# jwliao1209/DiffMusic

Measured on AMD Instinct MI355X. Metric: denoising steps/sec (10 s clip, 200-step DPS), higher is better.
Workload: dtype f16; 1 GPU; MusicLDM + DPS music_inpainting, 10 s @16 kHz, 200-step schedule, batch 8 per GPU (BASELINE.json configs[1]); global_batch=8, clips_per_gpu=8, lanes=1, parallelism=clip-sharded x1 (RCCL world size 1, no per-step collective), finite=True, nan_steps=0, settle_steps=10, cached_reference_transform=True, launched_by=single process

## Files before the change

diffmusic_amd/_lib.py:

```python
import ctypes as C
import os

_HERE = os.path.dirname(os.path.abspath(__file__))
LIB_PATH = os.environ.get("DMX_LIB_PATH") or os.path.join(_HERE, "lib", "libdiffmusic_hip.so")
MAX_STAGES = 8


class HifiGanConfig(C.Structure):
    _fields_ = [("model_in_dim", C.c_int), ("upsample_initial_channel", C.c_int), ("num_upsamples", C.c_int),
                ("upsample_rates", C.c_int * MAX_STAGES), ("upsample_kernel_sizes", C.c_int * MAX_STAGES),
                ("num_kernels", C.c_int), ("resblock_kernel_sizes", C.c_int * MAX_STAGES),
                ("num_dilations", C.c_int), ("resblock_dilation_sizes", C.c_int * (MAX_STAGES * MAX_STAGES)),
                ("leaky_relu_slope", C.c_float)]


class VaeConfig(C.Structure):
    _fields_ = [("latent_channels", C.c_int), ("out_channels", C.c_int), ("num_blocks", C.c_int),
                ("block_out_channels", C.c_int * MAX_STAGES), ("layers_per_block", C.c_int),
                ("norm_num_groups", C.c_int), ("eps", C.c_float)]


class UNetConfig(C.Structure):
    _fields_ = [("in_channels", C.c_int), ("out_channels", C.c_int), ("num_blocks", C.c_int),
                ("block_out_channels", C.c_int * MAX_STAGES), ("layers_per_block", C.c_int),
                ("attention_heads", C.c_int), ("norm_num_groups", C.c_int),
                ("down_attn", C.c_int * MAX_STAGES), ("up_attn", C.c_int * MAX_STAGES),
                ("class_embed_dim", C.c_int), ("num_attn_per_layer", C.c_int), ("attn_cross_dims", C.c_int * 4)]


class HtsatConfig(C.Structure):
    _fields_ = [("spec_size", C.c_int), ("num_mel_bins", C.c_int), ("patch_size", C.c_int), ("embed_dim", C.c_int), ("window_size", C.c_int),
                ("num_stages", C.c_int), ("depths", C.c_int * 4), ("num_heads", C.c_int * 4), ("ln_eps", C.c_float), ("bn_eps", C.c_float)]


class GemmDesc(C.Structure):
    _fields_ = [("A", C.c_void_p), ("W", C.c_void_p), ("C", C.c_void_p), ("C2", C.c_void_p),
                ("bias", C.c_void_p), ("rowbias", C.c_void_p), ("R", C.c_void_p), ("X", C.c_void_p),
                ("M", C.c_int), ("N", C.c_int), ("K", C.c_int), ("ldw", C.c_int),
                ("Hi", C.c_int), ("Wi", C.c_int), ("Ci", C.c_int), ("lda", C.c_int),
                ("Hq", C.c_int), ("Wq", C.c_int), ("sy", C.c_int), ("sx", C.c_int),
                ("ntaps", C.c_int),
                ("Ho", C.c_int), ("Wo", C.c_int), ("ldc", C.c_int), ("osy", C.c_int), ("ooy", C.c_int),
                ("osx", C.c_int), ("oox", C.c_int),
                ("ldr", C.c_int), ("ldx", C.c_int), ("ldc2", C.c_int),
                ("Z", C.c_int), ("Zi", C.c_int),
                ("sAo", C.c_longlong), ("sAi", C.c_longlong), ("sWo", C.c_longlong), ("sWi", C.c_longlong),
                ("sCo", C.c_longlong), ("sCi", C.c_longlong),
                ("alpha", C.c_float), ("act_slope", C.c_float), ("mask_slope", C.c_float),
                ("flags", C.c_int),
                ("tdy", C.c_byte * 16), ("tdx", C.c_byte * 16), ("resid_inv_slope", C.c_float), ("tile_cfg", C.c_int), ("ldrb", C.c_int), ("ksplit", C.c_int),
                ("XB", C.c_void_p), ("B2", C.c_void_p), ("ldxb", C.c_int), ("ldb2", C.c_int),
                ("colsum", C.c_void_p), ("ln_eps", C.c_float), ("rowstats_in", C.c_void_p), ("rowstats_out", C.c_void_p), ("nslots", C.c_int),
                ("gn_part", C.c_void_p), ("gnb_x", C.c_void_p), ("gnb_scale", C.c_void_p), ("gnb_shift", C.c_void_p),
                ("gnb_ldx", C.c_int), ("gnb_silu", C.c_int), ("gnb_stats", C.c_void_p), ("gnb_cpg", C.c_int)]


EPI_BIAS, EPI_ROWBIAS, EPI_RESID, EPI_ACCUM, EPI_MASK, EPI_LRELU2, EPI_TANH, EPI_F32OUT, EPI_NO_C, EPI_RESID_INV, EPI_MASKBITS, EPI_BITS2, EPI_SOFTBWD = \
    1, 2, 4, 8, 16, 32, 64, 128, 256, 512, 1024, 2048, 4096
EPI_GEGLU, EPI_LNFOLD, EPI_ROWSTATS, EPI_GNSTATS, EPI_GNBWD = 8192, 16384, 32768, 65536, 131072

_SIGS = {
    "dmx_abi_version": (C.c_int, []),
    "dmx_act_dtype": (C.c_int, []),
    "dmx_last_error": (C.c_char_p, []),
    "dmx_hifigan_create": (C.c_void_p, [C.POINTER(HifiGanConfig)]),
    "dmx_vae_decoder_create": (C.c_void_p, [C.POINTER(VaeConfig)]),
    "dmx_unet_create": (C.c_void_p, [C.POINTER(UNetConfig)]),
    "dmx_model_destroy": (None, [C.c_void_p]),
    "dmx_model_num_params": (C.c_int, [C.c_void_p]),
    "dmx_model_param_name": (C.c_char_p, [C.c_void_p, C.c_int]),
    "dmx_model_param_numel": (C.c_size_t, [C.c_void_p, C.c_int]),
    "dmx_model_param_ndim": (C.c_int, [C.c_void_p, C.c_int]),
    "dmx_model_param_dim": (C.c_int, [C.c_void_p, C.c_int, C.c_int]),
    "dmx_model_load_param": (C.c_int, [C.c_void_p, C.c_char_p, C.c_void_p, C.c_size_t]),
    "dmx_model_finalize": (C.c_int, [C.c_void_p, C.c_void_p]),
    "dmx_hifigan_out_len": (C.c_int, [C.c_void_p, C.c_int]),
    "dmx_hifigan_workspace_bytes": (C.c_size_t, [C.c_void_p, C.c_int, C.c_int]),
    "dmx_hifigan_fwd": (C.c_int, [C.c_void_p, C.c_void_p, C.c_void_p, C.c_int, C.c_int, C.c_void_p, C.c_size_t, C.c_void_p]),
    "dmx_hifigan_bwd": (C.c_int, [C.c_void_p, C.c_void_p, C.c_void_p, C.c_void_p]),
    "dmx_hifigan_fwd_dead": (C.c_int, [C.c_void_p, C.c_void_p, C.c_void_p, C.c_int, C.c_int, C.c_int, C.c_int, C.c_void_p, C.c_size_t,
                                       C.c_void_p]),
    "dmx_hifigan_dead_plan": (C.c_int, [C.c_void_p, C.POINTER(C.c_int), C.POINTER(C.c_int), C.POINTER(C.c_int), C.POINTER(C.c_int), C.c_int]),
    "dmx_conv_dead_rows": (C.c_int, [C.c_int] * 9 + [C.POINTER(C.c_int), C.POINTER(C.c_int)]),
    "dmx_vae_workspace_bytes": (C.c_size_t, [C.c_void_p, C.c_int, C.c_int, C.c_int]),
    "dmx_vae_decode_fwd": (C.c_int, [C.c_void_p, C.c_void_p, C.c_float, C.c_void_p, C.c_void_p, C.c_int, C.c_int, C.c_int,
                                     C.c_int, C.c_void_p, C.c_size_t, C.c_void_p]),
    "dmx_vae_decode_bwd": (C.c_int, [C.c_void_p, C.c_void_p, C.c_float, C.c_void_p, C.c_void_p]),
    "dmx_vae_encoder_create": (C.c_void_p, [C.POINTER(VaeConfig)]),
    "dmx_vae_encoder_workspace_bytes": (C.c_size_t, [C.c_void_p, C.c_int, C.c_int, C.c_int]),
    "dmx_vae_encode_fwd": (C.c_int, [C.c_void_p, C.c_void_p, C.c_float, C.c_void_p, C.c_int, C.c_int, C.c_int, C.c_void_p, C.c_size_t,
                                     C.c_void_p]),
    "dmx_latent_init": (C.c_int, [C.c_void_p] * 6 + [C.c_int] * 3 + [C.c_float] * 3 + [C.c_void_p]),
    "dmx_conv2d_raw": (C.c_int, [C.c_void_p] * 4 + [C.c_int] * 9 + [C.c_void_p]),
    "dmx_unet_workspace_bytes": (C.c_size_t, [C.c_void_p, C.c_int, C.c_int, C.c_int]),
    "dmx_unet_fwd": (C.c_int, [C.c_void_p, C.c_void_p, C.c_void_p, C.c_void_p, C.c_void_p, C.c_int, C.c_int, C.c_int,
                               C.c_void_p, C.c_size_t, C.c_void_p]),
    "dmx_unet_fwd_ctx": (C.c_int, [C.c_void_p] * 5 + [C.c_int, C.c_void_p, C.c_int, C.c_void_p, C.c_void_p, C.c_int, C.c_int, C.c_int,
                                   C.c_void_p, C.c_size_t, C.c_void_p]),
    "dmx_unet_workspace_bytes_ctx": (C.c_size_t, [C.c_void_p, C.c_int, C.c_int, C.c_int, C.c_int, C.c_int]),
    "dmx_htsat_create": (C.c_void_p, [C.POINTER(HtsatConfig)]),
    "dmx_htsat_feature_dims": (C.c_int, [C.c_void_p, C.POINTER(C.c_int), C.POINTER(C.c_int)]),
    "dmx_htsat_workspace_bytes": (C.c_size_t, [C.c_void_p, C.c_int, C.c_int]),
    "dmx_htsat_fwd": (C.c_int, [C.c_void_p, C.c_void_p, C.c_int, C.c_int, C.c_void_p, C.c_int, C.c_void_p, C.c_size_t, C.c_void_p]),
    "dmx_htsat_bwd": (C.c_int, [C.c_void_p, C.c_void_p, C.c_void_p, C.c_void_p, C.c_void_p]),
    "dmx_htsat_tape_raw": (C.c_size_t, [C.c_void_p, C.c_int, C.c_int, C.c_int, C.c_void_p, C.c_size_t, C.c_void_p]),
    "dmx_htsat_ln_rows_fwd_raw": (C.c_int, [C.c_void_p] * 4 + [C.c_longlong] + [C.c_int] * 4 + [C.c_float, C.c_int, C.c_void_p]),
    "dmx_htsat_ln_rows_bwd_raw": (C.c_int, [C.c_void_p] * 5 + [C.c_longlong] + [C.c_int] * 4 + [C.c_float, C.c_int, C.c_void_p]),
    "dmx_htsat_gelu_fwd_raw": (C.c_int, [C.c_void_p, C.c_void_p, C.c_longlong, C.c_void_p]),
    "dmx_htsat_gelu_bwd_raw": (C.c_int, [C.c_void_p, C.c_void_p, C.c_void_p, C.c_longlong, C.c_void_p]),
    "dmx_htsat_win_attn_fwd_raw": (C.c_int, [C.c_void_p] * 3 + [C.c_int] * 6 + [C.c_void_p]),
    "dmx_htsat_win_attn_bwd_raw": (C.c_int, [C.c_void_p] * 4 + [C.c_int] * 6 + [C.c_void_p]),
    "dmx_htsat_embed_fwd_raw": (C.c_int, [C.c_void_p, C.c_void_p, C.c_int, C.c_int, C.c_void_p, C.c_void_p]),
    "dmx_htsat_embed_bwd_raw": (C.c_int, [C.c_void_p, C.c_void_p, C.c_int, C.c_int] + [C.c_void_p] * 5),
    "dmx_gram_fwd": (C.c_int, [C.c_void_p, C.c_void_p, C.c_int, C.c_int, C.c_int, C.c_void_p]),
    "dmx_gram_bwd": (C.c_int, [C.c_void_p, C.c_void_p, C.c_void_p, C.c_int, C.c_int, C.c_int, C.c_void_p]),
    "dmx_gemm_raw": (C.c_int, [C.c_void_p, C.c_size_t, C.c_void_p]),
    "dmx_gemm_slab_eligible": (C.c_int, [C.c_void_p, C.c_size_t]),
    "dmx_gemm_last_cfg_raw": (C.c_int, []),
    "dmx_prof_begin": (None, []),
    "dmx_prof_end": (C.c_int, [C.POINTER(C.c_double), C.POINTER(C.c_double)]),
    "dmx_flash_attn_raw": (C.c_int, [C.c_void_p, C.c_void_p, C.c_void_p, C.c_void_p, C.c_void_p] + [C.c_int] * 6 + [C.c_float, C.c_void_p]),
    "dmx_flash_attn_ld_raw": (C.c_int, [C.c_void_p] * 5 + [C.c_int] * 8 + [C.c_float, C.POINTER(C.c_int), C.c_void_p]),
    "dmx_softmax_raw": (C.c_int, [C.c_void_p] * 3 + [C.c_longlong, C.c_int, C.c_longlong, C.c_longlong, C.c_int, C.c_void_p]),
    "dmx_softmax_act_raw": (C.c_int, [C.c_void_p] * 3 + [C.c_longlong, C.c_int, C.c_longlong, C.c_int, C.c_void_p]),
    "dmx_transpose_raw": (C.c_int, [C.c_void_p, C.c_void_p, C.c_int, C.c_int, C.c_longlong, C.c_longlong, C.c_int, C.c_int] + [C.c_longlong] * 4
                          + [C.c_void_p]),
    "dmx_rowdot_raw": (C.c_int, [C.c_void_p] * 3 + [C.c_longlong, C.c_int, C.c_longlong, C.c_longlong, C.c_void_p]),
    "dmx_layernorm_raw": (C.c_int, [C.c_void_p] * 4 + [C.c_int, C.c_int, C.c_float, C.c_void_p]),
    "dmx_geglu_raw": (C.c_int, [C.c_void_p, C.c_void_p, C.c_longlong, C.c_int, C.c_void_p]),
    "dmx_gemm_splitk_workspace": (C.c_int, [C.c_void_p, C.c_size_t]),
    "dmx_conv_pair_raw": (C.c_int, [C.c_void_p, C.c_void_p, C.c_size_t, C.c_void_p]),
    "dmx_conv_pair_group_raw": (C.c_int, [C.c_int, C.c_void_p, C.c_void_p, C.c_size_t, C.c_void_p]),
    "dmx_conv_pair_dead_raw": (C.c_int, [C.c_void_p, C.c_void_p, C.c_size_t, C.POINTER(C.c_int), C.POINTER(C.c_int), C.POINTER(C.c_int), C.c_void_p]),
    "dmx_conv_pair_group_dead_raw": (C.c_int, [C.c_int, C.c_void_p, C.c_void_p, C.c_size_t, C.POINTER(C.c_int), C.c_void_p]),
    "dmx_groupnorm_scratch_floats": (C.c_size_t, [C.c_int, C.c_int, C.c_int]),
    "dmx_groupnorm_raw": (C.c_int, [C.c_void_p] * 8 + [C.c_int] * 4 + [C.c_float, C.c_int, C.c_void_p]),
    "dmx_groupnorm_part_floats": (C.c_size_t, [C.c_int, C.c_int, C.c_int]),
    "dmx_groupnorm_parts_raw": (C.c_int, [C.c_void_p] * 7 + [C.c_int] * 4 + [C.c_float, C.c_int, C.c_int, C.c_void_p, C.c_void_p, C.c_void_p]),
    "dmx_gemm_last_tile_rows_raw": (C.c_int, []),
    "dmx_groupnorm_bwd_raw": (C.c_int, [C.c_void_p] * 10 + [C.c_int] * 6 + [C.c_void_p, C.c_void_p, C.c_void_p]),
    "dmx_prof_dominant": (C.c_int, [C.POINTER(C.c_double)] * 3),
    "dmx_audio_create": (C.c_void_p, [C.c_int, C.c_int, C.c_int, C.c_int, C.c_void_p]),
    "dmx_audio_destroy": (None, [C.c_void_p]),
    "dmx_audio_num_frames": (C.c_int, [C.c_void_p, C.c_int]),
    "dmx_audio_num_bins": (C.c_int, [C.c_void_p]),
    "dmx_audio_state_bytes": (C.c_size_t, [C.c_void_p, C.c_int, C.c_int]),
    "dmx_audio_transform_fwd": (C.c_int, [C.c_void_p, C.c_void_p, C.c_longlong, C.c_void_p, C.c_void_p, C.c_int, C.c_int, C.c_int,
                                          C.c_int, C.c_float, C.c_float, C.c_void_p]),
    "dmx_audio_transform_bwd": (C.c_int, [C.c_void_p, C.c_void_p, C.c_void_p, C.c_longlong, C.c_void_p, C.c_int, C.c_int, C.c_int,
                                          C.c_int, C.c_float, C.c_float, C.c_int, C.c_void_p]),
    "dmx_audio_is_fused": (C.c_int, [C.c_void_p, C.c_int]),
    "dmx_audio_guidance_fwd": (C.c_int, [C.c_void_p, C.c_void_p, C.c_longlong, C.c_void_p, C.c_void_p, C.c_longlong, C.c_void_p, C.c_void_p,
                                         C.c_int, C.c_int, C.c_int, C.c_int, C.c_float, C.c_float, C.c_void_p]),
    "dmx_audio_guidance_bwd": (C.c_int, [C.c_void_p, C.c_void_p, C.c_longlong, C.c_void_p, C.c_void_p, C.c_longlong, C.c_float, C.c_void_p,
                                         C.c_void_p, C.c_longlong, C.c_int, C.c_void_p, C.c_int, C.c_int, C.c_int, C.c_int, C.c_float, C.c_float,
                                         C.c_void_p]),
    "dmx_audio_guidance_fwd_ex": (C.c_int, [C.c_void_p, C.c_void_p, C.c_longlong, C.c_void_p, C.c_void_p, C.c_longlong, C.c_void_p, C.c_void_p,
                                            C.c_int, C.c_int, C.c_int, C.c_int, C.c_float, C.c_float, C.c_void_p, C.c_longlong, C.c_void_p,
                                            C.c_float, C.c_void_p]),
    "dmx_audio_guidance_bwd_ex": (C.c_int, [C.c_void_p, C.c_void_p, C.c_longlong, C.c_void_p, C.c_void_p, C.c_longlong, C.c_float, C.c_void_p,
                                            C.c_void_p, C.c_longlong, C.c_int, C.c_void_p, C.c_int, C.c_int, C.c_int, C.c_int, C.c_float, C.c_float,
                                            C.c_void_p, C.c_longlong, C.c_void_p, C.c_float, C.c_void_p]),
    "dmx_audio_guidance_fwd_shaped": (C.c_int, [C.c_void_p, C.c_void_p, C.c_longlong, C.c_void_p, C.c_void_p, C.c_longlong, C.c_void_p, C.c_void_p,
                                                C.c_int, C.c_int, C.c_int, C.c_int, C.c_float, C.c_float, C.c_void_p, C.c_longlong, C.c_void_p,
                                                C.c_float, C.c_void_p, C.c_void_p]),
    "dmx_audio_guidance_bwd_shaped": (C.c_int, [C.c_void_p, C.c_void_p, C.c_longlong, C.c_void_p, C.c_void_p, C.c_longlong, C.c_float, C.c_void_p,
                                                C.c_void_p, C.c_longlong, C.c_int, C.c_void_p, C.c_int, C.c_int, C.c_int, C.c_int, C.c_float, C.c_float,
                                                C.c_void_p, C.c_longlong, C.c_void_p, C.c_float, C.c_void_p, C.c_void_p]),
    "dmx_clip_fwd": (C.c_int, [C.c_void_p, C.c_longlong, C.c_void_p, C.c_void_p, C.c_longlong, C.c_int, C.c_int, C.c_void_p]),
    "dmx_clip_bwd": (C.c_int, [C.c_void_p, C.c_longlong, C.c_void_p, C.c_longlong, C.c_void_p, C.c_void_p, C.c_longlong, C.c_int, C.c_int, C.c_int,
                               C.c_void_p]),
    "dmx_declip_project": (C.c_int, [C.c_void_p, C.c_longlong, C.c_void_p, C.c_longlong, C.c_void_p, C.c_void_p, C.c_longlong, C.c_int, C.c_int,
                                     C.c_void_p]),
    "dmx_drc_fwd": (C.c_int, [C.c_void_p, C.c_longlong, C.c_void_p, C.c_longlong, C.c_void_p, C.c_void_p, C.c_int, C.c_int] + [C.c_float] * 6 +
                    [C.c_void_p]),
    "dmx_drc_bwd": (C.c_int, [C.c_void_p, C.c_longlong, C.c_void_p, C.c_longlong, C.c_void_p, C.c_void_p, C.c_void_p, C.c_void_p, C.c_longlong,
                              C.c_int, C.c_int, C.c_int] + [C.c_float] * 6 + [C.c_void_p]),
    "dmx_drc_fwd_p": (C.c_int, [C.c_void_p, C.c_longlong, C.c_void_p, C.c_longlong, C.c_void_p, C.c_void_p, C.c_void_p, C.c_int, C.c_int, C.c_float,
                                C.c_void_p]),
    "dmx_drc_bwd_p": (C.c_int, [C.c_void_p, C.c_longlong, C.c_void_p, C.c_longlong] + [C.c_void_p] * 6 + [C.c_longlong, C.c_int, C.c_int, C.c_int,
                                                                                                        C.c_float, C.c_void_p]),
    "dmx_drc_pgrad": (C.c_int, [C.c_void_p] * 6 + [C.c_int, C.c_int, C.c_float, C.c_void_p]),
    "dmx_drc_update": (C.c_int, [C.c_void_p] * 5 + [C.c_int] * 3 + [C.c_void_p] + [C.c_double] * 3 + [C.c_float, C.c_void_p, C.c_void_p, C.c_void_p]),
    "dmx_warp_fwd": (C.c_int, [C.c_void_p, C.c_longlong, C.c_void_p, C.c_longlong, C.c_void_p, C.c_int, C.c_int, C.c_void_p]),
    "dmx_warp_bwd": (C.c_int, [C.c_void_p, C.c_void_p, C.c_longlong, C.c_void_p, C.c_int, C.c_int, C.c_int, C.c_void_p]),
    "dmx_warp_wgrad": (C.c_int, [C.c_void_p, C.c_void_p, C.c_longlong, C.c_void_p, C.c_longlong, C.c_void_p, C.c_int, C.c_int, C.c_void_p]),
    "dmx_warp_update": (C.c_int, [C.c_void_p] * 5 + [C.c_int] * 4 + [C.c_double] * 5 + [C.c_int, C.c_void_p]),
    "dmx_click_detect": (C.c_int, [C.c_void_p, C.c_longlong] + [C.c_void_p] * 5 + [C.c_int, C.c_int, C.c_float, C.c_float, C.c_void_p]),
    "dmx_click_mask": (C.c_int, [C.c_void_p, C.c_void_p, C.c_void_p, C.c_int, C.c_int, C.c_int, C.c_void_p]),
    "dmx_mask_rows": (C.c_int, [C.c_void_p, C.c_longlong, C.c_void_p, C.c_longlong, C.c_void_p, C.c_int, C.c_int, C.c_int, C.c_void_p]),
    "dmx_declick_blend": (C.c_int, [C.c_void_p, C.c_longlong, C.c_void_p, C.c_longlong, C.c_void_p, C.c_longlong, C.c_void_p, C.c_int, C.c_int,
                                    C.c_int, C.c_void_p]),
    "dmx_noise_add": (C.c_int, [C.c_void_p, C.c_void_p, C.c_void_p, C.c_longlong, C.c_float, C.c_void_p]),
    "dmx_audio_stft_mag": (C.c_int, [C.c_void_p, C.c_void_p, C.c_longlong, C.c_void_p, C.c_void_p, C.c_int, C.c_int, C.c_void_p]),
    "dmx_audio_stft_mag_bwd": (C.c_int, [C.c_void_p, C.c_void_p, C.c_void_p, C.c_longlong, C.c_void_p, C.c_int, C.c_int, C.c_int, C.c_void_p]),
    "dmx_audio_tf_frames": (C.c_int, [C.c_int]),
    "dmx_audio_tf_gain": (C.c_int, [C.c_void_p, C.c_void_p, C.c_longlong, C.c_void_p, C.c_longlong, C.c_void_p, C.c_longlong, C.c_int, C.c_int, C.c_int,
                                    C.c_void_p]),
    "dmx_audio_tf_curve": (C.c_int, [C.c_void_p, C.c_void_p, C.c_longlong, C.c_void_p, C.c_longlong, C.c_void_p, C.c_longlong, C.c_int, C.c_int, C.c_int,
                                     C.c_void_p]),
    "dmx_audio_tf_wgrad_segments": (C.c_int, [C.c_int]),
    "dmx_audio_tf_wgrad": (C.c_int, [C.c_void_p, C.c_void_p, C.c_longlong, C.c_void_p, C.c_longlong, C.c_void_p, C.c_int, C.c_int, C.c_void_p]),
    "dmx_audio_eq_update": (C.c_int, [C.c_void_p, C.c_int] + [C.c_void_p] * 3 + [C.c_int, C.c_int] + [C.c_double] * 4 + [C.c_int, C.c_void_p]),
    "dmx_mdct_frames": (C.c_int, [C.c_int]),
    "dmx_mdct_quant": (C.c_int, [C.c_void_p, C.c_void_p, C.c_longlong, C.c_void_p, C.c_longlong, C.c_void_p, C.c_void_p, C.c_longlong, C.c_int, C.c_int,
                                 C.c_int, C.c_int, C.c_void_p]),
    "dmx_mdct_project": (C.c_int, [C.c_void_p, C.c_void_p, C.c_longlong, C.c_void_p, C.c_longlong, C.c_void_p, C.c_void_p, C.c_longlong, C.c_int,
                                   C.c_int, C.c_int, C.c_void_p]),
    "dmx_audio_melscale": (C.c_int, [C.c_void_p, C.c_void_p, C.c_void_p, C.c_int, C.c_int, C.c_float, C.c_float, C.c_void_p]),
    "dmx_mask_apply": (C.c_int, [C.c_void_p, C.c_longlong, C.c_void_p, C.c_void_p, C.c_longlong, C.c_int, C.c_int, C.c_int, C.c_void_p]),
    "dmx_l2_loss": (C.c_int, [C.c_void_p, C.c_longlong, C.c_void_p, C.c_void_p, C.c_void_p, C.c_int, C.c_longlong, C.c_float, C.c_void_p]),
    "dmx_track_stitch_fwd": (C.c_int, [C.c_void_p, C.c_longlong, C.c_void_p, C.POINTER(C.c_int)] + [C.c_int] * 4 + [C.c_void_p]),
    "dmx_track_stitch_bwd": (C.c_int, [C.c_void_p, C.c_void_p, C.c_longlong, C.POINTER(C.c_int)] + [C.c_int] * 5 + [C.c_void_p]),
    "dmx_stem_mix_fwd": (C.c_int, [C.c_void_p, C.c_longlong, C.c_void_p, C.POINTER(C.c_float)] + [C.c_int] * 3 + [C.c_void_p]),
    "dmx_stem_mix_bwd": (C.c_int, [C.c_void_p, C.c_void_p, C.c_longlong, C.POINTER(C.c_float)] + [C.c_int] * 4 + [C.c_void_p]),
    "dmx_stem_project": (C.c_int, [C.c_void_p, C.c_longlong, C.c_void_p, C.c_void_p, C.POINTER(C.c_float), C.c_int, C.c_int, C.c_void_p]),
    "dmx_grad_normalize": (C.c_int, [C.c_void_p, C.c_void_p, C.c_int, C.c_longlong, C.c_float, C.c_void_p]),
    "dmx_fir_fwd": (C.c_int, [C.c_void_p, C.c_longlong, C.c_void_p, C.c_void_p, C.c_longlong] + [C.c_int] * 7 + [C.c_void_p]),
    "dmx_fir_bwd": (C.c_int, [C.c_void_p, C.c_longlong, C.c_void_p, C.c_void_p, C.c_void_p, C.c_longlong] + [C.c_int] * 7 + [C.c_void_p]),
    "dmx_fir_clip_fwd": (C.c_int, [C.c_void_p, C.c_longlong, C.c_void_p, C.c_void_p, C.c_longlong] + [C.c_int] * 4 + [C.c_void_p]),
    "dmx_fir_clip_bwd": (C.c_int, [C.c_void_p, C.c_longlong, C.c_void_p, C.c_void_p, C.c_void_p, C.c_longlong] + [C.c_int] * 4 + [C.c_void_p]),
    "dmx_fir_wgrad_workspace_floats": (C.c_size_t, [C.c_int, C.c_int, C.c_int]),
    "dmx_fir_wgrad": (C.c_int, [C.c_void_p, C.c_longlong, C.c_void_p, C.c_longlong, C.c_void_p, C.c_size_t] + [C.c_int] * 4 + [C.c_void_p]),
    "dmx_ir_update": (C.c_int, [C.c_void_p, C.c_int] + [C.c_void_p] * 4 + [C.c_int, C.c_int] + [C.c_double] * 4 + [C.c_int, C.c_void_p]),
    "dmx_sched_pred_x0": (C.c_int, [C.c_void_p, C.c_void_p, C.c_void_p, C.c_longlong, C.c_float, C.c_void_p]),
    "dmx_sched_pred_x0_ex": (C.c_int, [C.c_void_p, C.c_void_p, C.c_void_p, C.c_longlong, C.c_float, C.c_int, C.c_float, C.c_void_p]),
    "dmx_sched_step_ex": (C.c_int, [C.c_int] + [C.c_void_p] * 9 + [C.c_int, C.c_int] + [C.c_float] * 5 + [C.c_int, C.c_int, C.c_float, C.c_void_p]),
    "dmx_sched_cfg_combine": (C.c_int, [C.c_void_p, C.c_void_p, C.c_longlong, C.c_float, C.c_void_p]),
    "dmx_randn_philox": (C.c_int, [C.c_void_p, C.c_int, C.c_longlong, C.POINTER(C.c_ulonglong), C.c_ulonglong, C.c_void_p]),
    "dmx_sched_step": (C.c_int, [C.c_int] + [C.c_void_p] * 9 + [C.c_int, C.c_int] + [C.c_float] * 5 + [C.c_int, C.c_void_p]),
}

ADDED_IN_V4 = ("dmx_vae_encoder_create", "dmx_vae_encoder_workspace_bytes", "dmx_vae_encode_fwd", "dmx_latent_init",
               "dmx_track_stitch_fwd", "dmx_track_stitch_bwd", "dmx_audio_guidance_fwd_shaped", "dmx_audio_guidance_bwd_shaped",
               "dmx_clip_fwd", "dmx_clip_bwd", "dmx_declip_project", "dmx_hifigan_fwd_dead", "dmx_hifigan_dead_plan", "dmx_conv_dead_rows",
               "dmx_fir_clip_fwd", "dmx_fir_clip_bwd", "dmx_fir_wgrad", "dmx_fir_wgrad_workspace_floats", "dmx_ir_update",
               "dmx_stem_mix_fwd", "dmx_stem_mix_bwd", "dmx_stem_project", "dmx_audio_tf_gain", "dmx_audio_tf_frames",
               "dmx_audio_tf_curve", "dmx_audio_tf_wgrad_segments", "dmx_audio_tf_wgrad", "dmx_audio_eq_update", "dmx_drc_fwd", "dmx_drc_bwd",
               "dmx_warp_fwd", "dmx_warp_bwd", "dmx_warp_wgrad", "dmx_warp_update", "dmx_drc_fwd_p", "dmx_drc_bwd_p", "dmx_drc_pgrad",
               "dmx_drc_update", "dmx_click_detect", "dmx_click_mask", "dmx_mask_rows", "dmx_declick_blend", "dmx_mdct_frames",
               "dmx_mdct_quant", "dmx_mdct_project")

_lib = None


def check_symbols(h, path=LIB_PATH):
    for name in ADDED_IN_V4:
        if not hasattr(h, name):
            raise RuntimeError(f"{path} reports ABI version {ABI_VERSION} but does not export `{name}` (a build from before the VAE "
                               "encoder / track-mode / declipping / blind-dereverberation / source-separation / time-frequency-masking / blind-equalisation / de-compression / wow-and-flutter / blind-wow-and-flutter / blind-de-compression / declicking / codec-restoration entry points): rebuild it (python -m diffmusic_amd.build --force)")


def lib():
    global _lib
    if _lib is None:
        if not os.path.exists(LIB_PATH):
            raise RuntimeError(f"{LIB_PATH} is missing: build it with `python -m diffmusic_amd.build` "
                               "(the diffmusic_amd hot path has no CPU fallback)")
        h = C.CDLL(LIB_PATH)
        for name, (res, args) in _SIGS.items():
            if not hasattr(h, name):
                continue
            fn = getattr(h, name)
            fn.restype, fn.argtypes = res, args
        if h.dmx_abi_version() != ABI_VERSION:
            raise RuntimeError(f"libdiffmusic_hip.so ABI version {h.dmx_abi_version()} != {ABI_VERSION} expected by this package: rebuild it "
                               "(python -m diffmusic_amd.build --force)")
        check_symbols(h)
        _lib = h
    return _lib


ABI_VERSION = 4


def act_dtype():
    import torch
    return torch.float16 if lib().dmx_act_dtype() == 1 else torch.bfloat16


class DmxError(RuntimeError):
    pass


def check(rc, what=""):
    if rc != 0:
        msg = lib().dmx_last_error()
        raise DmxError(f"{what} failed with code {rc}: {msg.decode() if msg else ''}")
```

diffmusic_amd/csrc/blocks.h:

```cpp
#pragma once
#include <cstdlib>
#include "models.h"

struct Ctx {
  Arena* arena;
  hipStream_t st;
  bool dry;
  float* gn_partial;
  bool gn_parts = true;
};
#define CRUN(expr) do { if (!cx.dry) { int rc_ = (expr); if (rc_ != DMX_OK) return rc_; } } while (0)
#define CTRY(expr) do { int rc__ = (expr); if (rc__ != DMX_OK) return rc__; } while (0)

struct GnTape { float* stats = nullptr; float* scale = nullptr; float* shift = nullptr; };

inline bool gn_parts_wanted(const Ctx& cx, size_t P) {
  const bool on = cx.gn_parts && getenv("DMX_NO_GN_PARTS") == nullptr;
  return on && P > 512;
}
inline float* gn_part_alloc(Ctx& cx, int B, size_t P, int Np) { return cx.arena->f32(dmx_gn_part_floats(B, (int)P, Np)); }
inline void gn_parts_push(Ctx& cx, GnParts* gp, float* buf, int tm, int P, int Np, int Creal, int qoff = 0) {
  if (!gp || gp->n < 0) return;
  if (cx.dry) tm = 32;
  if (tm > 0 && gp->n < 8) gp->r[gp->n++] = GnRegion{buf, tm, P, Np / 4, qoff, Creal / 4};
  else gp->n = -1;
}
inline GnParts gn_parts_concat(const GnParts& a, const GnParts& b, int Ca) {
  GnParts o;
  if (a.n <= 0 || b.n <= 0 || a.n + b.n > 8) { o.n = -1; return o; }
  for (int i = 0; i < a.n; ++i) o.r[o.n++] = a.r[i];
  for (int i = 0; i < b.n; ++i) { o.r[o.n] = b.r[i]; o.r[o.n++].qoff += Ca / 4; }
  return o;
}
inline const GnParts* gn_parts_valid(const GnParts* p) { return p && p->n > 0 ? p : nullptr; }
inline GnParts gn_parts_new(Ctx& cx, int B, size_t P, int Np) {
  GnParts g;
  if (gn_parts_wanted(cx, P)) g.r[0].part = gn_part_alloc(cx, B, P, Np); else g.n = -1;
  return g;
}
inline float* gn_parts_buf(const GnParts& g) { return g.n == 0 ? g.r[0].part : nullptr; }

inline int conv_fwd_2d_gn(Ctx& cx, const ConvLayer& L, const act_t* in, void* out, int B, int H, int W, Epi e, GnParts* out_parts, int Creal) {
  float* buf = out_parts ? gn_parts_buf(*out_parts) : nullptr;
  e.gn_part = buf;
  int rows = 0;
  CRUN(conv_fwd_2d(L, in, out, B, H, W, e, cx.st, &rows));
  const int Ho = (H + L.pad_h + L.pad_h_hi - L.kh) / L.stride + 1, Wo = (W + L.pad_w + L.pad_w_hi - L.kw) / L.stride + 1;
  if (buf) gn_parts_push(cx, out_parts, buf, rows, Ho * Wo, L.Cop, Creal);
  return DMX_OK;
}

inline int upsample_conv_fwd_gn(Ctx& cx, const ConvLayer& L, const act_t* x, act_t* y, int B, int H, int W, int H2, int W2, int C, bool fold,
                                GnParts* out_parts) {
  Arena& A = *cx.arena;
  const size_t P = (size_t)H * W, P2 = (size_t)H2 * W2;
  GnParts up;
  float* ubuf[4] = {nullptr, nullptr, nullptr, nullptr};
  if (gn_parts_wanted(cx, P2)) for (int q = 0; q < (fold ? 4 : 1); ++q) ubuf[q] = gn_part_alloc(cx, B, fold ? P : P2, L.Cop);
  else up.n = -1;
  const size_t mk = A.mark();
  Epi e;
  if (fold) {
    int rows[4] = {0, 0, 0, 0};
    CRUN(conv_up2x_fwd(L, x, y, B, H, W, e, cx.st, ubuf[0] ? ubuf : nullptr, rows));
    if (ubuf[0]) for (int q = 0; q < 4; ++q) gn_parts_push(cx, &up, ubuf[q], rows[q], (int)P, L.Cop, C);
  } else {
    act_t* u = A.bf(B * P2 * C);
    CRUN(dmx_upsample_nearest(x, u, B, H, W, H2, W2, C, cx.st));
    up.r[0].part = ubuf[0];
    CTRY(conv_fwd_2d_gn(cx, L, u, y, B, H2, W2, e, &up, C));
  }
  A.release(mk);
  *out_parts = up;
  return DMX_OK;
}

struct GnLayer {
  GroupNormLayer g;
  const float* gamma = nullptr;
  const float* beta = nullptr;
  void build(ParamStore& ps, const std::string& pre, int C, int G, float eps) { g = make_gn(ps, pre, C, G, eps); }
  void bind(ParamStore& ps) { gamma = ps.dev(g.g_id); beta = ps.dev(g.b_id); }
  GnTape alloc(Ctx& cx, int B) const {
    GnTape t;
    t.stats = cx.arena->f32((size_t)B * g.G * 2);
    t.scale = cx.arena->f32((size_t)B * g.C);
    t.shift = cx.arena->f32((size_t)B * g.C);
    return t;
  }
  int fwd(Ctx& cx, const act_t* x, act_t* y, int B, int P, int silu, const GnTape& t, const GnParts* parts = nullptr) const {
    CRUN(dmx_groupnorm_fwd(x, y, gamma, beta, t.stats, t.scale, t.shift, cx.gn_partial, B, P, g.C, g.G, g.eps, silu, cx.st,
                           gn_parts_valid(parts)));
    return DMX_OK;
  }
  int conv_bwd_2d_gn(Ctx& cx, const ConvLayer& L, const act_t* dout, act_t* dy, int B, int H, int W, const act_t* x, int silu, const GnTape& t,
                     GnParts* bparts) const {
    const size_t P = (size_t)H * W;
    GnParts gp;
    Epi e;
    int rows = 0;
    if (!gn_parts_wanted(cx, P) || ((g.C / g.G) & 3) || (g.C & 7) || getenv("DMX_NO_GN_BWD_PARTS")) {
      gp.n = -1;
    } else {
      e.gn_part = gn_part_alloc(cx, B, P, g.C);
      e.gnb_x = x; e.gnb_scale = t.scale; e.gnb_shift = t.shift; e.gnb_silu = silu; e.gnb_stats = t.stats; e.gnb_cpg = g.C / g.G;
    }
    CRUN(conv_bwd_2d(L, dout, dy, B, H, W, e, cx.st, &rows));
    if (e.gn_part) gn_parts_push(cx, &gp, e.gn_part, rows, (int)P, g.C, g.C);
    *bparts = gp;
    return DMX_OK;
  }
  int bwd(Ctx& cx, const act_t* x, const act_t* dy, const act_t* add, act_t* dx, int B, int P, int silu, const GnTape& t,
          const GnParts* bparts = nullptr) const {
    const size_t mk = cx.arena->mark();
    float* k0 = cx.arena->f32((size_t)B * g.C);
    float* k1 = cx.arena->f32((size_t)B * g.C);
    CRUN(dmx_groupnorm_bwd(x, dy, add, dx, t.stats, t.scale, t.shift, k0, k1, cx.gn_partial, B, P, g.C, g.G, silu, cx.st,
                           gn_parts_valid(bparts)));
    cx.arena->release(mk);
    return DMX_OK;
  }
};

struct ResnetTape { const act_t* x = nullptr; act_t* h1 = nullptr; GnTape g1, g2; };

struct Resnet2D {
  int Cin = 0, Cout = 0;
  GnLayer norm1, norm2;
  ConvLayer conv1, conv2, shortcut, temb;
  bool has_shortcut = false, has_temb = false;

  void build(ParamStore& ps, const std::string& pre, int cin, int cout, int temb_ch, int groups, float eps, bool need_bwd) {
    Cin = cin; Cout = cout;
    norm1.build(ps, pre + ".norm1", cin, groups, eps);
    conv1 = make_conv2d(ps, pre + ".conv1", cin, cout, 3, 1, 1, need_bwd);
    if (temb_ch > 0) { temb = make_linear(ps, pre + ".time_emb_proj", temb_ch, cout, true, false); has_temb = true; }
    norm2.build(ps, pre + ".norm2", cout, groups, eps);
    conv2 = make_conv2d(ps, pre + ".conv2", cout, cout, 3, 1, 1, need_bwd);
    if (cin != cout) { shortcut = make_conv2d(ps, pre + ".conv_shortcut", cin, cout, 1, 1, 0, need_bwd); has_shortcut = true; }
  }
  int pack(ParamStore& ps, hipStream_t st) {
    norm1.bind(ps); norm2.bind(ps);
    CTRY(pack_layer(ps, conv1, st));
    CTRY(pack_layer(ps, conv2, st));
    if (has_shortcut) CTRY(pack_layer(ps, shortcut, st));
    if (has_temb) CTRY(pack_layer(ps, temb, st));
    return DMX_OK;
  }
  int fwd(Ctx& cx, const act_t* x, act_t* out, int B, int H, int W, const act_t* silu_emb, ResnetTape* tape,
          const float* rb_pre = nullptr, int ldrb = 0, const GnParts* x_parts = nullptr, GnParts* out_parts = nullptr) const {
    Arena& A = *cx.arena;
    const size_t P = (size_t)H * W;
    ResnetTape t;
    t.x = x;
    if (tape) { t.h1 = A.bf(B * P * Cout); t.g1 = norm1.alloc(cx, B); t.g2 = norm2.alloc(cx, B); }
    const size_t mk = A.mark();
    if (!tape) { t.h1 = A.bf(B * P * Cout); t.g1 = norm1.alloc(cx, B); t.g2 = norm2.alloc(cx, B); }
    act_t* n = A.bf(B * P * (Cin > Cout ? Cin : Cout));
    CTRY(norm1.fwd(cx, x, n, B, (int)P, 1, t.g1, x_parts));
    Epi e1;
    GnParts h1p = gn_parts_new(cx, B, P, conv1.Cop);
    if (has_temb && rb_pre) {
      e1.flags = EPI_ROWBIAS; e1.rowbias = rb_pre; e1.ldrb = ldrb;
    } else if (has_temb) {
      float* rb = A.f32((size_t)B * Cout);
      Epi et; et.flags = EPI_F32OUT;
      CRUN(linear_fwd(temb, silu_emb, temb.Cip, rb, Cout, B, et, cx.st));
      e1.flags = EPI_ROWBIAS; e1.rowbias = rb;
    }
    CTRY(conv_fwd_2d_gn(cx, conv1, n, t.h1, B, H, W, e1, &h1p, Cout));
    CTRY(norm2.fwd(cx, t.h1, n, B, (int)P, 1, t.g2, &h1p));
    Epi e2; e2.flags = EPI_RESID; e2.R = x;
    if (has_shortcut) {
      act_t* sc = A.bf(B * P * Cout);
      Epi es;
      CRUN(conv_fwd_2d(shortcut, x, sc, B, H, W, es, cx.st));
      e2.R = sc;
    }
    CTRY(conv_fwd_2d_gn(cx, conv2, n, out, B, H, W, e2, out_parts, Cout));
    A.release(mk);
    if (tape) *tape = t;
    return DMX_OK;
  }
  int bwd(Ctx& cx, const act_t* dout, act_t* dx, int B, int H, int W, const ResnetTape& t) const {
    Arena& A = *cx.arena;
    const size_t P = (size_t)H * W;
    const size_t mk = A.mark();
    act_t* a = A.bf(B * P * Cout);
    act_t* b = A.bf(B * P * (Cin > Cout ? Cin : Cout));
    Epi e;
    GnParts bp2, bp1;
    CTRY(norm2.conv_bwd_2d_gn(cx, conv2, dout, a, B, H, W, t.h1, 1, t.g2, &bp2));
    CTRY(norm2.bwd(cx, t.h1, a, nullptr, b, B, (int)P, 1, t.g2, &bp2));
    act_t* c = A.bf(B * P * Cin);
    CTRY(norm1.conv_bwd_2d_gn(cx, conv1, b, c, B, H, W, t.x, 1, t.g1, &bp1));
    const act_t* add = dout;
    if (has_shortcut) {
      CRUN(conv_bwd_2d(shortcut, dout, b, B, H, W, e, cx.st));
      add = b;
    }
    CTRY(norm1.bwd(cx, t.x, c, add, dx, B, (int)P, 1, t.g1, &bp1));
    A.release(mk);
    return DMX_OK;
  }
};

inline int attention_core(Ctx& cx, const act_t* q, const act_t* k, const act_t* v, act_t* o, int B, int Nq, int Nk, int C,
                          int heads, act_t* P_keep, const float* colbias, int ldq = 0, int ldk = 0, int ldv = 0) {
  if (ldq <= 0) ldq = C;
  if (ldk <= 0) ldk = C;
  if (ldv <= 0) ldv = C;
  Arena& A = *cx.arena;
  const int dh = C / heads, Z = B * heads;
  const int Nkp = pad8(Nk);
  if (dh & 7) { dmx_set_error("attention needs head_dim %% 8 == 0 (dh=%d)", dh); return DMX_ERR_SHAPE; }
  const float scale = 1.0f / sqrtf((float)dh);
  const size_t mk = A.mark();
  static const bool fused_ok = getenv("DMX_NO_FLASH") == nullptr;
  const bool flash = !P_keep && fused_ok && dmx_flash_attn_ok(dh, C);
  if (!flash && (Nk & 3)) { dmx_set_error("attention through materialised scores needs Nk %% 4 == 0 (Nk=%d)", Nk); return DMX_ERR_SHAPE; }
  if (flash) {
    CRUN(dmx_flash_attn_fwd(q, k, v, o, colbias, B, Nq, Nk, C, heads, scale, cx.st, ldq, ldk, ldv));
    A.release(mk);
    return DMX_OK;
  }
  act_t* Pm = P_keep ? P_keep : A.bf((size_t)Z * Nq * Nkp);
  act_t* vT = A.bf((size_t)Z * dh * Nkp);
  GemmBatch gb;
  gb.Z = Z; gb.Zi = heads;
  gb.sAo = (long long)Nq * ldq; gb.sAi = dh;
  gb.sBo = (long long)Nk * ldk; gb.sBi = dh;
  gb.sCo = (long long)heads * Nq * Nkp; gb.sCi = (long long)Nq * Nkp;
  Epi e; e.alpha = scale;
  CRUN(gemm_nt(q, ldq, k, ldk, Pm, Nkp, Nq, Nk, dh, e, gb, cx.st));
  CRUN(dmx_softmax_act(Pm, Pm, colbias, (long long)Z * Nq, Nk, Nkp, heads * Nq, cx.st));
  if (Nkp != Nk && !cx.dry) (void)hipMemsetAsync(vT, 0, (size_t)Z * dh * Nkp * sizeof(act_t), cx.st);
  CRUN(dmx_transpose(v, vT, Nk, dh, ldv, Nkp, Z, heads, (long long)Nk * ldv, dh, (long long)heads * dh * Nkp, (long long)dh * Nkp, cx.st));
  GemmBatch g2;
  g2.Z = Z; g2.Zi = heads;
  g2.sAo = (long long)heads * Nq * Nkp; g2.sAi = (long long)Nq * Nkp;
  g2.sBo = (long long)heads * dh * Nkp; g2.sBi = (long long)dh * Nkp;
  g2.sCo = (long long)Nq * C; g2.sCi = dh;
  Epi e2;
  CRUN(gemm_nt(Pm, Nkp, vT, Nkp, o, C, Nq, dh, Nkp, e2, g2, cx.st));
  A.release(mk);
  return DMX_OK;
}

struct VaeMidAttention {
  int C = 0;
  bool need_bwd = false;
  GnLayer norm;
  ConvLayer to_q, to_k, to_v, to_out;
  GnTape t_norm;
  const act_t* x_in = nullptr;
  act_t *q = nullptr, *k = nullptr, *v = nullptr, *Pm = nullptr, *O = nullptr;

  void build(ParamStore& ps, const std::string& pre, int C_, int G, float eps, bool need_bwd_) {
    C = C_; need_bwd = need_bwd_;
    norm.build(ps, pre + ".group_norm", C, G, eps);
    to_q = make_linear(ps, pre + ".to_q", C, C, true, need_bwd);
    to_k = make_linear(ps, pre + ".to_k", C, C, true, need_bwd);
    to_v = make_linear(ps, pre + ".to_v", C, C, true, need_bwd);
    to_out = make_linear(ps, pre + ".to_out.0", C, C, true, need_bwd);
  }
  int pack(ParamStore& ps, hipStream_t st) {
    norm.bind(ps);
    CTRY(pack_layer(ps, to_q, st));
    CTRY(pack_layer(ps, to_k, st));
    CTRY(pack_layer(ps, to_v, st));
    CTRY(pack_layer(ps, to_out, st));
    return DMX_OK;
  }
  int fwd(Ctx& cx, const act_t* x, act_t** out, int B, int H, int W, bool keep, const GnParts* x_parts, GnParts* out_parts) {
    Arena& A = *cx.arena;
    const int N = H * W;
    const size_t n = (size_t)B * N * C;
    x_in = x;
    t_norm = norm.alloc(cx, B);
    if (need_bwd) { q = A.bf(n); k = A.bf(n); v = A.bf(n); }
    Pm = keep ? A.bf((size_t)B * N * pad8(N)) : nullptr;
    O = keep ? A.bf(n) : nullptr;
    act_t* y = A.bf(n);
    GnParts op = gn_parts_new(cx, B, (size_t)N, pad8(C));
    const size_t mk = A.mark();
    act_t* xn = A.bf(n);
    if (!need_bwd) { q = A.bf(n); k = A.bf(n); v = A.bf(n); }
    act_t* o = keep ? O : A.bf(n);
    CTRY(norm.fwd(cx, x, xn, B, N, 0, t_norm, x_parts));
    Epi e;
    CRUN(linear_fwd(to_q, xn, C, q, C, (long long)B * N, e, cx.st));
    CRUN(linear_fwd(to_k, xn, C, k, C, (long long)B * N, e, cx.st));
    CRUN(linear_fwd(to_v, xn, C, v, C, (long long)B * N, e, cx.st));
    CTRY(attention_core(cx, q, k, v, o, B, N, N, C, 1, Pm, nullptr));
    Epi er; er.flags = EPI_RESID; er.R = x;
    if (gn_parts_buf(op)) CTRY(conv_fwd_2d_gn(cx, to_out, o, y, B, H, W, er, &op, C));
    else CRUN(linear_fwd(to_out, o, C, y, C, (long long)B * N, er, cx.st));
    A.release(mk);
    *out = y; *out_parts = op;
    return DMX_OK;
  }
  int bwd(Ctx& cx, const act_t* g, act_t* gx, int B, int H, int W) const {
    Arena& A = *cx.arena;
    const int N = H * W;
    hipStream_t st = cx.st;
    if (N & 7) { dmx_set_error("vae attention backward needs h*w %% 8 == 0"); return DMX_ERR_SHAPE; }
    if ((long long)B * N * C >= (1ll << 29)) { dmx_set_error("vae attention backward: B*h*w*C >= 2^29 elements unsupported"); return DMX_ERR_SHAPE; }
    const float scale = 1.0f / sqrtf((float)C);
    const size_t mk = A.mark();
    act_t* go = A.bf((size_t)B * N * C);
    act_t* goT = A.bf((size_t)B * N * C);
    act_t* PT = A.bf((size_t)B * N * N);
    float* delta = A.f32((size_t)B * N);
    act_t* dS = A.bf((size_t)B * N * N);
    act_t* T1 = A.bf((size_t)B * N * C);
    act_t* gq = A.bf((size_t)B * N * C);
    act_t* gk = A.bf((size_t)B * N * C);
    act_t* gv = A.bf((size_t)B * N * C);
    act_t* gxn = A.bf((size_t)B * N * C);
    Epi e;
    CRUN(linear_bwd(to_out, g, C, go, C, (long long)B * N, e, st));
    GemmBatch gb; gb.Z = B; gb.Zi = 1;
    CRUN(dmx_rowdot(go, O, delta, (long long)B * N, C, C, C, st));
    gb.sAo = (long long)N * C; gb.sBo = (long long)N * C; gb.sCo = (long long)N * N;
    {
      Epi es; es.flags = EPI_SOFTBWD; es.X = Pm; es.rowbias = delta; es.alpha = scale;
      CRUN(gemm_nt(go, C, v, C, dS, N, N, N, C, es, gb, st));
    }
    CRUN(dmx_transpose(Pm, PT, N, N, N, N, B, 1, (long long)N * N, 0, (long long)N * N, 0, st));
    CRUN(dmx_transpose(go, goT, N, C, C, N, B, 1, (long long)N * C, 0, (long long)N * C, 0, st));
    gb.sAo = (long long)N * N; gb.sBo = (long long)N * C; gb.sCo = (long long)N * C;
    CRUN(gemm_nt(PT, N, goT, N, gv, C, N, C, N, e, gb, st));
    CRUN(dmx_transpose(k, T1, N, C, C, N, B, 1, (long long)N * C, 0, (long long)N * C, 0, st));
    CRUN(gemm_nt(dS, N, T1, N, gq, C, N, C, N, e, gb, st));
    CRUN(dmx_transpose(dS, PT, N, N, N, N, B, 1, (long long)N * N, 0, (long long)N * N, 0, st));
    CRUN(dmx_transpose(q, T1, N, C, C, N, B, 1, (long long)N * C, 0, (long long)N * C, 0, st));
    CRUN(gemm_nt(PT, N, T1, N, gk, C, N, C, N, e, gb, st));
    Epi ea; ea.flags = EPI_ACCUM;
    CRUN(linear_bwd(to_q, gq, C, gxn, C, (long long)B * N, e, st));
    CRUN(linear_bwd(to_k, gk, C, gxn, C, (long long)B * N, ea, st));
    CRUN(linear_bwd(to_v, gv, C, gxn, C, (long long)B * N, ea, st));
    CTRY(norm.bwd(cx, x_in, gxn, g, gx, B, N, 0, t_norm));
    A.release(mk);
    return DMX_OK;
  }
};
```

diffmusic_amd/csrc/dmx_common.h:

```cpp
#pragma once
#include <hip/hip_runtime.h>
#include <stdint.h>
#include <stddef.h>

typedef uint16_t act_t;

#define DMX_OK 0
#define DMX_ERR_SHAPE (-1)
#define DMX_ERR_WORKSPACE (-2)
#define DMX_ERR_PARAM (-3)
#define DMX_ERR_STATE (-4)
#define DMX_ERR_LAUNCH (-5)

typedef __attribute__((ext_vector_type(4))) float f32x4;
#ifdef DMX_BF16
typedef __bf16 native16_t;
typedef __attribute__((ext_vector_type(8))) __bf16 frag8_t;
#define DMX_MFMA16(a, b, c) __builtin_amdgcn_mfma_f32_16x16x32_bf16(a, b, c, 0, 0, 0)
#define DMX_ACT_DTYPE 0
#else
typedef _Float16 native16_t;
typedef __attribute__((ext_vector_type(8))) _Float16 frag8_t;
#define DMX_MFMA16(a, b, c) __builtin_amdgcn_mfma_f32_16x16x32_f16(a, b, c, 0, 0, 0)
#define DMX_ACT_DTYPE 1
#endif

__device__ __forceinline__ float a2f(act_t v) { return (float)__builtin_bit_cast(native16_t, v); }
__device__ __forceinline__ act_t f2a(float f) { return __builtin_bit_cast(act_t, (native16_t)f); }
#ifdef DMX_BF16
__device__ __forceinline__ uint32_t pack2a(float lo, float hi) { return (uint32_t)f2a(lo) | ((uint32_t)f2a(hi) << 16); }
#else
__device__ __forceinline__ uint32_t pack2a(float lo, float hi) {
  typedef float dmx_f32x2 __attribute__((ext_vector_type(2)));
  typedef _Float16 dmx_f16x2 __attribute__((ext_vector_type(2)));
  const dmx_f32x2 v = {lo, hi};
  return __builtin_bit_cast(uint32_t, __builtin_convertvector(v, dmx_f16x2));
}
#endif
__device__ __forceinline__ float alo(uint32_t u) { return a2f((act_t)(u & 0xffffu)); }
__device__ __forceinline__ float ahi(uint32_t u) { return a2f((act_t)(u >> 16)); }

__device__ __forceinline__ float wave_sum(float v) {
#pragma unroll
  for (int o = 32; o > 0; o >>= 1) v += __shfl_xor(v, o, 64);
  return v;
}
__device__ __forceinline__ float wave_max(float v) {
#pragma unroll
  for (int o = 32; o > 0; o >>= 1) v = fmaxf(v, __shfl_xor(v, o, 64));
  return v;
}
__device__ __forceinline__ float block_sum(float v, float* sh) {
  v = wave_sum(v);
  const int w = threadIdx.x >> 6, nw = blockDim.x >> 6;
  __syncthreads();
  if ((threadIdx.x & 63) == 0) sh[w] = v;
  __syncthreads();
  float r = 0.f;
  for (int i = 0; i < nw; ++i) r += sh[i];
  return r;
}
__device__ __forceinline__ float block_max(float v, float* sh) {
  v = wave_max(v);
  const int w = threadIdx.x >> 6, nw = blockDim.x >> 6;
  __syncthreads();
  if ((threadIdx.x & 63) == 0) sh[w] = v;
  __syncthreads();
  float r = -3.0e38f;
  for (int i = 0; i < nw; ++i) r = fmaxf(r, sh[i]);
  return r;
}

static inline int cdiv(int a, int b) { return (a + b - 1) / b; }
static inline size_t align_up(size_t v, size_t a) { return (v + a - 1) / a * a; }

#define DMX_MAX_TAPS 16
enum {
  EPI_BIAS = 1,
  EPI_ROWBIAS = 2,
  EPI_RESID = 4,
  EPI_ACCUM = 8,
  EPI_MASK = 16,
  EPI_LRELU2 = 32,
  EPI_TANH = 64,
  EPI_F32OUT = 128,
  EPI_NO_C = 256,
  EPI_RESID_INV = 512,
  EPI_MASKBITS = 1024,
  EPI_BITS2 = 2048,
  EPI_GEGLU = 8192,
  EPI_LNFOLD = 16384,
  EPI_ROWSTATS = 32768,
  EPI_GNSTATS = 65536,
  EPI_GNBWD = 131072,
  EPI_BIASINIT = 262144,
  EPI_SOFTBWD = 4096
};

struct GemmDesc {
  const act_t* A;
  const act_t* W;
  void* C;
  act_t* C2;
  const float* bias;
  const float* rowbias;
  const act_t* R;
  const act_t* X;
  int M, N, K;
  int ldw;
  int Hi, Wi, Ci, lda;
  int Hq, Wq, sy, sx;
  int ntaps;
  int Ho, Wo, ldc, osy, ooy, osx, oox;
  int ldr, ldx, ldc2;
  int Z, Zi;
  long long sAo, sAi, sWo, sWi, sCo, sCi;
  float alpha, act_slope, mask_slope;
  int flags;
  signed char tdy[DMX_MAX_TAPS], tdx[DMX_MAX_TAPS];
  float resid_inv_slope;
  int tile_cfg;
  int ldrb;
  int ksplit;
  const unsigned char* XB;
  unsigned char* B2;
  int ldxb, ldb2;
  const float* colsum;
  float ln_eps;
  const float* rowstats_in;
  float* rowstats_out;
  int nslots;
  float* gn_part;
  const act_t* gnb_x;
  const float* gnb_scale;
  const float* gnb_shift;
  int gnb_ldx, gnb_silu;
  const float* gnb_stats;
  int gnb_cpg;
};

int dmx_gemm_launch(const GemmDesc& d, hipStream_t stream, int* gn_rows = nullptr);
void dmx_gemm_set_splitk_workspace(float* ws, size_t bytes);
void dmx_gemm_release_splitk_workspace(const float* ws);
int dmx_gemm_launch_ln(int cfg, const GemmDesc& d, hipStream_t stream);
int dmx_gemm_launch_rowstats(int cfg, const GemmDesc& d, hipStream_t stream);
int dmx_gemm_launch_gnstats(int cfg, const GemmDesc& d, hipStream_t stream, int* gn_rows);
bool dmx_prof_is_active();
bool dmx_gemm_slab_ok(const GemmDesc& d);
int dmx_gemm_last_cfg();
```

diffmusic_amd/csrc/gemm_conv.hip:

```cpp
#include "gemm_tile.h"

namespace {
template <int BM, int BN, int WM, int WN, int NSTAGE>
int launch_glds(const GemmDesc& d, hipStream_t stream) {
  if (d.flags & EPI_SOFTBWD) {
    if constexpr (BM == 256 && BN == 256) return launch_glds_t<BM, BN, WM, WN, NSTAGE, 2>(d, stream);
    else return DMX_ERR_SHAPE;
  }
  if (d.flags & EPI_GEGLU) return launch_glds_t<BM, BN, WM, WN, NSTAGE, 3>(d, stream);
  return (d.flags & (EPI_MASKBITS | EPI_BITS2)) ? launch_glds_t<BM, BN, WM, WN, NSTAGE, 1>(d, stream)
                                                : launch_glds_t<BM, BN, WM, WN, NSTAGE, 0>(d, stream);
}

template <int S>
int launch_slab(const GemmDesc& d, hipStream_t stream) {
  return (d.flags & (EPI_MASKBITS | EPI_BITS2)) ? launch_glds_t<320, 256, 2, 4, 2, 1, false, S>(d, stream)
                                                : launch_glds_t<320, 256, 2, 4, 2, 0, false, S>(d, stream);
}

template <int BM, int BN, int WM, int WN>
int launch_cfg(const GemmDesc& d, hipStream_t stream) {
  if (d.flags & EPI_SOFTBWD) return DMX_ERR_SHAPE;
  if (d.flags & EPI_GEGLU) {
    if constexpr ((BN / WN) % 32 == 0) return launch_cfg_t<BM, BN, WM, WN, 3>(d, stream);
    else return DMX_ERR_SHAPE;
  }
  return (d.flags & (EPI_MASKBITS | EPI_BITS2)) ? launch_cfg_t<BM, BN, WM, WN, 1>(d, stream) : launch_cfg_t<BM, BN, WM, WN, 0>(d, stream);
}

}

#include <vector>
#include <cstdio>
#include <cstdlib>
#include <cmath>
namespace {
struct ProfRec { hipEvent_t a, b; double flops, bytes; int M, N, K, Z, taps, flags, cfg; };
int g_last_cfg = 0;
bool g_prof = false;
std::vector<ProfRec> g_prof_recs;
struct TileEntry { int M, N, K, Z, cfg; };
static const TileEntry g_tile_table[] = {
#include "tile_table.inc"
    {0, 0, 0, 0, 0}};

bool glds_ok(const GemmDesc& d) {
  const long long imgs = d.Hq * d.Wq > 0 ? (d.M + (long long)d.Hq * d.Wq - 1) / ((long long)d.Hq * d.Wq) : 1;
  const long long in_elems = (d.Hi > 1 || d.ntaps > 1 ? imgs * d.Hi * d.Wi : (long long)d.M) * d.lda;
  static const bool strided_ok = getenv("DMX_NO_GLDS_STRIDED") == nullptr;
  return in_elems < (1ll << 29) && (long long)d.M * d.lda < (1ll << 29) && ((long long)d.N + 512) * d.ldw < (1ll << 29) &&
         (d.sy == 1 || strided_ok);
}
}

bool dmx_gemm_slab_ok(const GemmDesc& d) {
  if (d.Hi != 1 || d.Hq != 1 || d.sx != 1 || d.ntaps < 2 || d.ntaps > DMX_MAX_TAPS || (d.Ci & 63) || d.Ci <= 0 || d.N <= 0 || (d.N & 255)) return false;
  if (d.Wq <= 0 || d.M % d.Wq != 0 || d.ksplit > 1) return false;
  int lo = 127, hi = -128;
  for (int t = 0; t < d.ntaps; ++t) {
    if (d.tdy[t] != 0) return false;
    lo = d.tdx[t] < lo ? d.tdx[t] : lo;
    hi = d.tdx[t] > hi ? d.tdx[t] : hi;
  }
  if (hi - lo > SLAB_HALO) return false;
  if (d.flags & (EPI_F32OUT | EPI_SOFTBWD | EPI_GEGLU | EPI_LNFOLD | EPI_ROWSTATS | EPI_GNSTATS | EPI_GNBWD)) return false;
  if ((d.ldc | d.ldr | d.ldx | d.ldc2) & 7) return false;
  return glds_ok(d);
}
int dmx_gemm_last_cfg() { return g_last_cfg; }

namespace {
inline int slab_cfg(int ntaps) { return ntaps >= 6 ? 21 : (ntaps >= 3 ? 20 : 22); }
int slab_adopt(const GemmDesc& d) {
  static const bool no_slab = getenv("DMX_NO_SLAB") != nullptr;
  if (no_slab || !(d.N == 256 || d.N == 512) || !(d.ntaps == 3 || d.ntaps == 7 || d.ntaps == 11) || d.Z != 1 || !dmx_gemm_slab_ok(d)) return 7;
  const long long flat = (long long)cdiv(d.M, 320) * (d.N / 256), per_image = (long long)(d.M / d.Wq) * cdiv(d.Wq, 320) * (d.N / 256);
  return (per_image + 255) / 256 <= (flat + 255) / 256 ? slab_cfg(d.ntaps) : 7;
}

int launch_by_cfg(int cfg, const GemmDesc& d, hipStream_t stream, int* gn_rows = nullptr) {
  g_last_cfg = cfg;
  if (cfg >= 20 && cfg <= 22) {
    const int S = cfg == 20 ? 2 : (cfg == 21 ? 1 : 3);
    if (!dmx_gemm_slab_ok(d) || d.ntaps * S < 6) return DMX_ERR_SHAPE;
    return S == 2 ? launch_slab<2>(d, stream) : (S == 1 ? launch_slab<1>(d, stream) : launch_slab<3>(d, stream));
  }
  if (d.flags & EPI_LNFOLD) return dmx_gemm_launch_ln(cfg, d, stream);
  if (d.flags & EPI_ROWSTATS) return dmx_gemm_launch_rowstats(cfg, d, stream);
  if (d.flags & (EPI_GNSTATS | EPI_GNBWD)) return dmx_gemm_launch_gnstats(cfg, d, stream, gn_rows);
  switch (cfg) {
    case 1: return launch_glds<256, 256, 2, 4, 2>(d, stream);
    case 2: return launch_glds<256, 128, 4, 2, 3>(d, stream);
    case 7: return launch_glds<320, 256, 2, 4, 2>(d, stream);
    case 8: return launch_glds<192, 256, 2, 4, 2>(d, stream);
    case 9: return launch_glds<320, 128, 4, 2, 2>(d, stream);
    case 10: return launch_glds<192, 128, 4, 2, 3>(d, stream);
    case 11: return launch_glds<128, 128, 2, 2, 2>(d, stream);
    case 12: return launch_glds<64, 64, 2, 2, 4>(d, stream);
    case 13: return launch_glds<128, 64, 2, 2, 3>(d, stream);
    case 14: return launch_glds<64, 128, 2, 2, 3>(d, stream);
    case 15: return launch_glds<64, 64, 2, 2, 8>(d, stream);
    case 16: return launch_glds<64, 128, 2, 2, 6>(d, stream);
    case 17: return launch_glds<128, 64, 2, 2, 6>(d, stream);
    case 18: return launch_glds<128, 128, 2, 2, 4>(d, stream);
    case 19: return launch_glds<512, 128, 4, 2, 2>(d, stream);
    case 3: return launch_cfg<128, 128, 2, 2>(d, stream);
    case 4: return launch_cfg<128, 64, 2, 2>(d, stream);
    case 5: return launch_cfg<128, 32, 4, 1>(d, stream);
    default: return launch_cfg<64, 64, 2, 2>(d, stream);
  }
}
int launch_dispatch(const GemmDesc& d, hipStream_t stream, int* gn_rows) {
  const bool gl = glds_ok(d);
  if (d.flags & EPI_SOFTBWD) return gl ? launch_by_cfg(1, d, stream, gn_rows) : DMX_ERR_SHAPE;
  if (d.tile_cfg >= 1 && d.tile_cfg <= 22 && ((d.tile_cfg > 2 && d.tile_cfg < 7) || gl)) return launch_by_cfg(d.tile_cfg, d, stream, gn_rows);
  {
    static int ovN[8], ovC[8], nov = -1;
    if (nov < 0) {
      nov = 0;
      if (const char* e = getenv("DMX_CFG_OVERRIDE")) {
        while (*e && nov < 8) {
          int n = 0, c = 0;
          if (sscanf(e, "%d:%d", &n, &c) == 2) { ovN[nov] = n; ovC[nov] = c; ++nov; }
          while (*e && *e != ',') ++e;
          if (*e == ',') ++e;
        }
      }
    }
    if (gl && d.M >= 40000)
      for (int i = 0; i < nov; ++i) if (ovN[i] == d.N) return launch_by_cfg(ovC[i], d, stream, gn_rows);
  }
  for (const TileEntry* e = g_tile_table; e->cfg; ++e)
    if (e->M == d.M && e->N == d.N && e->K == d.K && e->Z == d.Z) {
      int c = e->cfg % 100;
      if (c == 7) c = slab_adopt(d);
      if ((c > 2 && c < 7) || gl) return launch_by_cfg(c, d, stream, gn_rows);
    }
  if (gl && d.M >= 2048 && d.N % 128 == 0) {
    auto cost = [&](int bm, int bn, int slots, double eff) {
      const double blocks = (double)cdiv(d.M, bm) * cdiv(d.N, bn) * d.Z;
      const double rounds = ceil(blocks / slots);
      return rounds * (bm / 128.0) * (bn / 128.0) * (slots / 256.0) / eff;
    };
    struct Cand { int cfg, bm, bn, slots; double eff; };
    static const Cand cands[] = {{1, 256, 256, 256, 0.95}, {7, 320, 256, 256, 0.93}, {8, 192, 256, 256, 0.88},
                                 {2, 256, 128, 256, 0.70}, {9, 320, 128, 256, 0.70}, {10, 192, 128, 256, 0.66},
                                 {19, 512, 128, 256, 0.75},
                                 {3, 128, 128, 512, 0.66}};
    int best = 0;
    double bc = 1e30;
    for (const Cand& c : cands) {
      if (c.bn == 256 && d.N % 256) continue;
      const double v = cost(c.bm, c.bn, c.slots, c.eff);
      if (v < bc) { bc = v; best = c.cfg; }
    }
    if (best == 7) best = slab_adopt(d);
    if (best && best != 3) return launch_by_cfg(best, d, stream, gn_rows);
  }
  if (d.N > 32 && (long long)cdiv(d.M, 128) * cdiv(d.N, 128) * d.Z < 200) {
    if (gl && d.K >= 512 && d.Z == 1) return launch_by_cfg(d.N % 128 == 0 && d.M >= 4000 ? 14 : 12, d, stream, gn_rows);
    return launch_by_cfg(6, d, stream, gn_rows);
  }
  if (d.N > 64) return launch_by_cfg(3, d, stream, gn_rows);
  if (d.N > 32) return launch_by_cfg(4, d, stream, gn_rows);
  return launch_by_cfg(5, d, stream, gn_rows);
}
}

bool dmx_prof_is_active() { return g_prof; }

extern "C" void dmx_prof_begin(void) {
  for (auto& r : g_prof_recs) { (void)hipEventDestroy(r.a); (void)hipEventDestroy(r.b); }
  g_prof_recs.clear();
  g_prof = true;
}
static double g_dma_ms = 0.0, g_dma_fl = 0.0, g_dma_by = 0.0;
static int g_dma_n = 0;
#ifdef DMX_GEMM_STAMPS
extern "C" int dmx_gemm_stamps_read(unsigned long long* host) {
  return hipMemcpyFromSymbol(host, HIP_SYMBOL(g_gemm_stamps), sizeof(unsigned long long) * 8192 * 6) == hipSuccess ? 0 : -1;
}
#endif

extern "C" int dmx_prof_dominant(double* ms, double* flops, double* bytes) {
  if (ms) *ms = g_dma_ms;
  if (flops) *flops = g_dma_fl;
  if (bytes) *bytes = g_dma_by;
  return g_dma_n;
}
extern "C" int dmx_prof_end(double* total_ms, double* total_flops) {
  g_prof = false;
  g_dma_ms = g_dma_fl = g_dma_by = 0.0; g_dma_n = 0;
  (void)hipDeviceSynchronize();
  double ms = 0.0, fl = 0.0;
  FILE* csv = getenv("DMX_PROF_CSV") ? fopen(getenv("DMX_PROF_CSV"), "w") : nullptr;
  if (csv) fprintf(csv, "M,N,K,Z,taps,flags,cfg,ms,tflops\n");
  for (auto& r : g_prof_recs) {
    float t = 0.f;
    if (hipEventElapsedTime(&t, r.a, r.b) == hipSuccess) ms += t;
    if (csv) fprintf(csv, "%d,%d,%d,%d,%d,%d,%d,%.4f,%.1f\n", r.M, r.N, r.K, r.Z, r.taps, r.flags, r.cfg, t, t > 0 ? r.flops / t / 1e9 : 0.0);
    const bool dma = r.cfg == 1 || r.cfg == 2 || (r.cfg >= 7 && r.cfg <= 10) || (r.cfg >= 19 && r.cfg <= 22);
    if (dma) { g_dma_ms += t; g_dma_fl += r.flops; g_dma_by += r.bytes; ++g_dma_n; }
    fl += r.flops;
    (void)hipEventDestroy(r.a); (void)hipEventDestroy(r.b);
  }
  if (csv) fclose(csv);
  const int n = (int)g_prof_recs.size();
  g_prof_recs.clear();
  if (total_ms) *total_ms = ms;
  if (total_flops) *total_flops = fl;
  return n;
}

namespace {
float* g_splitk_ws = nullptr;
size_t g_splitk_bytes = 0;

__global__ void splitk_epilogue_kernel(const GemmDesc p, const float* __restrict__ ws, int ksplit) {
  const long long q = (long long)blockIdx.x * blockDim.x + threadIdx.x;
  const int nq = p.N >> 2;
  if (q >= (long long)p.M * nq) return;
  const int m = (int)(q / nq), n = (int)(q - (long long)m * nq) * 4;
  const long long mn = (long long)p.M * p.N;
  float4 v = *reinterpret_cast<const float4*>(ws + (long long)m * p.N + n);
  for (int s = 1; s < ksplit; ++s) {
    const float4 w = *reinterpret_cast<const float4*>(ws + s * mn + (long long)m * p.N + n);
    v.x += w.x; v.y += w.y; v.z += w.z; v.w += w.w;
  }
  float a[4] = {v.x, v.y, v.z, v.w};
  const int flags = p.flags;
  const long long row = m;
  if (flags & EPI_MASK) {
    const uint2 xr = *reinterpret_cast<const uint2*>(p.X + row * p.ldx + n);
    const float x[4] = {alo(xr.x), ahi(xr.x), alo(xr.y), ahi(xr.y)};
#pragma unroll
    for (int e = 0; e < 4; ++e) a[e] *= x[e] > 0.f ? 1.f : p.mask_slope;
  }
  if (flags & EPI_BIAS) {
    const float4 bb = *reinterpret_cast<const float4*>(p.bias + n);
    a[0] += bb.x; a[1] += bb.y; a[2] += bb.z; a[3] += bb.w;
  }
  if (flags & EPI_ROWBIAS) {
    const float4 bb = *reinterpret_cast<const float4*>(p.rowbias + (long long)(m / (p.Hq * p.Wq)) * (p.ldrb ? p.ldrb : p.N) + n);
    a[0] += bb.x; a[1] += bb.y; a[2] += bb.z; a[3] += bb.w;
  }
  if (flags & EPI_RESID) {
    const uint2 rr = *reinterpret_cast<const uint2*>(p.R + row * p.ldr + n);
    const float is = (flags & EPI_RESID_INV) ? p.resid_inv_slope : 1.f;
    const float x[4] = {alo(rr.x), ahi(rr.x), alo(rr.y), ahi(rr.y)};
#pragma unroll
    for (int e = 0; e < 4; ++e) a[e] += fminf(x[e], x[e] * is);
  }
#pragma unroll
  for (int e = 0; e < 4; ++e) a[e] *= p.alpha;
  if (!(flags & EPI_NO_C))
    *reinterpret_cast<uint2*>(reinterpret_cast<act_t*>(p.C) + row * p.ldc + n) = make_uint2(pack2a(a[0], a[1]), pack2a(a[2], a[3]));
  if (flags & EPI_LRELU2) {
    const float sl = p.act_slope;
    *reinterpret_cast<uint2*>(p.C2 + row * p.ldc2 + n) =
        make_uint2(pack2a(fmaxf(a[0], a[0] * sl), fmaxf(a[1], a[1] * sl)), pack2a(fmaxf(a[2], a[2] * sl), fmaxf(a[3], a[3] * sl)));
  }
}

int splitk_plan(const GemmDesc& d, int* tile) {
  static const bool off = getenv("DMX_NO_SPLITK") != nullptr;
  if (off || !g_splitk_ws || d.Z != 1 || !glds_ok(d)) return 1;
  if (d.flags & (EPI_ACCUM | EPI_F32OUT | EPI_TANH | EPI_MASKBITS | EPI_BITS2 | EPI_SOFTBWD | EPI_GEGLU | EPI_LNFOLD | EPI_ROWSTATS)) return 1;
  if (!(d.osy == 1 && d.osx == 1 && d.ooy == 0 && d.oox == 0 && d.Ho == d.Hq && d.Wo == d.Wq)) return 1;
  if ((d.N & 7) || (d.ldc & 3)) return 1;
  const int nk = (d.K + BK - 1) / BK;
  auto fits = [&](int ks) { return ks >= 2 && ks <= nk && (size_t)ks * d.M * d.N * sizeof(float) <= g_splitk_bytes; };
  auto dma_tile = [](int t) { return t == 1 || t == 2 || (t >= 7 && t <= 19); };
  if (d.tile_cfg >= 100) { *tile = d.tile_cfg % 100; return fits(d.tile_cfg / 100) && dma_tile(*tile) ? d.tile_cfg / 100 : 1; }
  if (d.tile_cfg) return 1;
  for (const TileEntry* e = g_tile_table; e->cfg; ++e)
    if (e->M == d.M && e->N == d.N && e->K == d.K && e->Z == d.Z) {
      if (e->cfg < 100) return 1;
      *tile = e->cfg % 100;
      return fits(e->cfg / 100) && dma_tile(*tile) ? e->cfg / 100 : 1;
    }
  if (d.M > 8192) return 1;
  const long long tiles = (long long)cdiv(d.M, 64) * cdiv(d.N, 64);
  if (nk < 24 || tiles >= 256) return 1;
  int ks = (int)(1024 / tiles);
  if (ks > nk / 8) ks = nk / 8;
  if (ks > 8) ks = 8;
  while (ks > 1 && !fits(ks)) --ks;
  *tile = d.N % 128 == 0 && d.M >= 4096 ? 14 : 12;
  return ks < 2 ? 1 : ks;
}

int launch_splitk(const GemmDesc& d, int ks, int tile, hipStream_t stream) {
  GemmDesc g = d;
  g.ksplit = ks;
  g.flags = EPI_F32OUT;
  g.C = g_splitk_ws; g.C2 = nullptr; g.ldc = d.N; g.alpha = 1.f;
  g.bias = nullptr; g.rowbias = nullptr; g.R = nullptr; g.X = nullptr;
  g.Ho = d.Hq; g.Wo = d.Wq;
  g.tile_cfg = 0;
  int rc = launch_by_cfg(tile, g, stream);
  if (rc != DMX_OK) return rc;
  const long long nthr = (long long)d.M * (d.N >> 2);
  hipLaunchKernelGGL(splitk_epilogue_kernel, dim3((unsigned)((nthr + 255) / 256)), dim3(256), 0, stream, d, g_splitk_ws, ks);
  g_last_cfg = 100 * ks + tile;
  return hipGetLastError() == hipSuccess ? DMX_OK : DMX_ERR_LAUNCH;
}
}

void dmx_gemm_set_splitk_workspace(float* ws, size_t bytes) { g_splitk_ws = ws; g_splitk_bytes = bytes; }
void dmx_gemm_release_splitk_workspace(const float* ws) { if (g_splitk_ws == ws) { g_splitk_ws = nullptr; g_splitk_bytes = 0; } }

int dmx_prof_open(hipStream_t st) {
  if (!g_prof) return -1;
  ProfRec r;
  memset(&r, 0, sizeof(r));
  (void)hipEventCreate(&r.a); (void)hipEventCreate(&r.b);
  (void)hipEventRecord(r.a, st);
  g_prof_recs.push_back(r);
  return (int)g_prof_recs.size() - 1;
}
void dmx_prof_close(int rec, hipStream_t st, double flops, double bytes, int M, int N, int K, int taps, int flags, int cfg) {
  if (rec < 0 || rec >= (int)g_prof_recs.size()) return;
  ProfRec& r = g_prof_recs[rec];
  (void)hipEventRecord(r.b, st);
  r.flops = flops; r.bytes = bytes; r.M = M; r.N = N; r.K = K; r.Z = 1; r.taps = taps; r.flags = flags; r.cfg = cfg;
}

int dmx_gemm_launch(const GemmDesc& d, hipStream_t stream, int* gn_rows) {
  if (gn_rows) *gn_rows = 0;
  if (d.M <= 0 || d.N <= 0 || d.K <= 0) return DMX_ERR_SHAPE;
  if ((d.Ci & 7) || (d.N & 3) || (d.K & 7) || (d.lda & 7) || (d.ldw & 7) || (d.ldc & 3)) return DMX_ERR_SHAPE;
  if (d.ntaps < 1 || d.ntaps > DMX_MAX_TAPS || d.K != d.ntaps * d.Ci) return DMX_ERR_SHAPE;
  if (d.Z < 1 || d.Zi < 1) return DMX_ERR_SHAPE;
  if ((d.flags & EPI_LRELU2) && !(d.act_slope >= 0.f && d.act_slope <= 1.f)) return DMX_ERR_SHAPE;
  if ((d.flags & EPI_RESID_INV) && !(d.resid_inv_slope >= 1.f)) return DMX_ERR_SHAPE;
  if (d.flags & EPI_SOFTBWD) {
    if ((d.flags & ~(EPI_SOFTBWD)) || ((d.N | d.ldc | d.ldx) & 7) || !d.X || !d.rowbias || d.Zi != 1 || d.ntaps != 1) return DMX_ERR_SHAPE;
    if (!(d.osy == 1 && d.osx == 1 && d.ooy == 0 && d.oox == 0 && d.Ho == d.Hq && d.Wo == d.Wq)) return DMX_ERR_SHAPE;
  }
  if (d.flags & EPI_GEGLU) {
    if ((d.flags & ~(EPI_GEGLU | EPI_BIAS | EPI_LNFOLD)) || (d.N & 31) || (d.ldc & 7) || d.ldc < d.N / 2 || d.alpha != 1.f) return DMX_ERR_SHAPE;
    if ((d.ldr | d.ldx | d.ldc2) & 7) return DMX_ERR_SHAPE;
    if (!(d.osy == 1 && d.osx == 1 && d.ooy == 0 && d.oox == 0 && d.Ho == d.Hq && d.Wo == d.Wq)) return DMX_ERR_SHAPE;
  }
  if (d.flags & (EPI_MASKBITS | EPI_BITS2)) {
    if ((d.flags & EPI_F32OUT) || ((d.N | d.ldc | d.ldr | d.ldx | d.ldc2) & 7) || d.Z != 1) return DMX_ERR_SHAPE;
    if ((d.flags & EPI_MASKBITS) && (!d.XB || d.ldxb * 8 < d.N)) return DMX_ERR_SHAPE;
    if ((d.flags & EPI_BITS2) && (!d.B2 || d.ldb2 * 8 < d.N)) return DMX_ERR_SHAPE;
  }
  if ((d.flags & EPI_LNFOLD) && (d.flags & EPI_BIAS)) {
    GemmDesc q = d;
    q.flags &= ~EPI_BIAS;
    return dmx_gemm_launch(q, stream, gn_rows);
  }
  if (d.flags & EPI_LNFOLD) {
    if (d.ntaps != 1 || d.K != d.Ci || !d.colsum || !d.rowstats_in || d.nslots < 1 || d.Z != 1 ||
        (d.flags & (EPI_F32OUT | EPI_MASK | EPI_MASKBITS | EPI_BITS2 | EPI_SOFTBWD | EPI_ACCUM | EPI_TANH | EPI_LRELU2 | EPI_ROWSTATS)))
      return DMX_ERR_SHAPE;
  }
  if (d.flags & EPI_ROWSTATS) {
    if (!d.rowstats_out || d.nslots * 32 != d.N || d.Z != 1 || ((d.ldc | d.ldr) & 7) ||
        (d.flags & (EPI_F32OUT | EPI_MASK | EPI_MASKBITS | EPI_BITS2 | EPI_SOFTBWD | EPI_ACCUM | EPI_TANH | EPI_LRELU2 | EPI_GEGLU | EPI_NO_C)))
      return DMX_ERR_SHAPE;
    if (!(d.osy == 1 && d.osx == 1 && d.ooy == 0 && d.oox == 0 && d.Ho == d.Hq && d.Wo == d.Wq)) return DMX_ERR_SHAPE;
  }
  if (d.flags & (EPI_GNSTATS | EPI_GNBWD)) {
    bool can = d.gn_part && d.Z == 1 && !(d.flags & (EPI_F32OUT | EPI_NO_C | EPI_GEGLU | EPI_SOFTBWD | EPI_MASKBITS | EPI_BITS2 | EPI_LNFOLD | EPI_ROWSTATS | EPI_LRELU2)) &&
               !((d.N | d.ldc | d.ldr | d.ldx | d.ldc2) & 7) && (d.flags & (EPI_GNSTATS | EPI_GNBWD)) != (EPI_GNSTATS | EPI_GNBWD);
    if (d.flags & EPI_GNBWD) can = can && d.gnb_x && d.gnb_scale && d.gnb_shift && d.gnb_stats && !(d.gnb_ldx & 7) && d.gnb_cpg >= 4 && !(d.gnb_cpg & 3) && d.N % d.gnb_cpg == 0;
    int kt = 12;
    if (!can || splitk_plan(d, &kt) > 1) { GemmDesc q = d; q.flags &= ~(EPI_GNSTATS | EPI_GNBWD); return dmx_gemm_launch(q, stream, gn_rows); }
  }
  int ktile = 12;
  const int ksp = splitk_plan(d, &ktile);
  if (ksp <= 1 && d.tile_cfg >= 100) return DMX_ERR_SHAPE;
  if (!g_prof) return ksp > 1 ? launch_splitk(d, ksp, ktile, stream) : launch_dispatch(d, stream, gn_rows);
  ProfRec r;
  (void)hipEventCreate(&r.a); (void)hipEventCreate(&r.b);
  r.flops = 2.0 * d.M * (double)d.N * d.K * d.Z;
  {
    const double mn = (double)d.M * d.N * d.Z;
    double by = 2.0 * d.M * (double)d.Ci * d.Z + 2.0 * d.N * (double)d.K * (d.sWo ? d.Z : 1);
    if (!(d.flags & EPI_NO_C)) by += mn * ((d.flags & EPI_F32OUT) ? 4.0 : 2.0);
    if (d.flags & EPI_ACCUM) by += mn * ((d.flags & EPI_F32OUT) ? 4.0 : 2.0);
    if (d.flags & (EPI_RESID | EPI_RESID_INV)) by += mn * 2.0;
    if (d.flags & (EPI_MASK | EPI_SOFTBWD)) by += mn * 2.0;
    if (d.flags & EPI_MASKBITS) by += mn / 8.0;
    if (d.flags & EPI_BITS2) by += mn / 8.0;
    if (d.C2 && (d.flags & EPI_LRELU2)) by += mn * 2.0;
    r.bytes = by;
  }
  r.M = d.M; r.N = d.N; r.K = d.K; r.Z = d.Z; r.taps = d.ntaps; r.flags = d.flags;
  (void)hipEventRecord(r.a, stream);
  const int rc = ksp > 1 ? launch_splitk(d, ksp, ktile, stream) : launch_dispatch(d, stream, gn_rows);
  (void)hipEventRecord(r.b, stream);
  r.cfg = g_last_cfg;
  g_prof_recs.push_back(r);
  return rc;
}
```

diffmusic_amd/csrc/gemm_tile.h:

```cpp
#pragma once
#include "dmx_common.h"
#include <type_traits>
#include <cstdlib>

#include "gemm_epilogue.h"
#include "conv_pair.h"

namespace {

constexpr int BK = 64;
constexpr int DMX_DEF_BIG = 0;

template <int BM, int BN, int NT>
__device__ __forceinline__ void ln_prologue(const GemmDesc& p, int m0, int n0, float2* s_ln, float* s_cs) {
  constexpr int TPR = NT / BM >= 4 ? 4 : (NT / BM >= 2 ? 2 : 1);
  const int tid = threadIdx.x, ns = p.nslots;
  const int r = tid / TPR, sub = tid - r * TPR;
  const float inv_c = 1.f / (float)p.K;
  if (r < BM) {
    const int m = m0 + r;
    const bool row_ok = m < p.M;
    const float2* rs = reinterpret_cast<const float2*>(p.rowstats_in) + (long long)(row_ok ? m : 0) * ns;
    float si = 0.f, qi = 0.f;
    for (int t0 = 0; t0 < ns; t0 += TPR * 8) {
      float2 v[8];
#pragma unroll
      for (int u = 0; u < 8; ++u) {
        const int t = t0 + u * TPR + sub;
        v[u] = (row_ok && t < ns) ? rs[t] : make_float2(0.f, 0.f);
      }
#pragma unroll
      for (int u = 0; u < 8; ++u) { si += v[u].x; qi += v[u].y; }
    }
    if constexpr (TPR >= 2) { si += __shfl_xor(si, 1, 64); qi += __shfl_xor(qi, 1, 64); }
    if constexpr (TPR >= 4) { si += __shfl_xor(si, 2, 64); qi += __shfl_xor(qi, 2, 64); }
    const float mean = si * inv_c;
    if (sub == 0) s_ln[r] = make_float2(mean, rsqrtf(fmaxf(qi * inv_c - mean * mean, 0.f) + p.ln_eps));
  }
  for (int c = tid; c < BN; c += NT) {
    const bool ok = n0 + c < p.N;
    s_cs[c] = ok ? p.colsum[n0 + c] : 0.f;
    s_cs[BN + c] = (ok && p.bias) ? p.bias[n0 + c] : 0.f;
  }
}
template <int FM, int FN, int BN>
__device__ __forceinline__ void ln_apply(f32x4 (&acc)[FM][FN], const float2* s_ln, const float* s_cs, int r0, int c0, int lr, int lq) {
#pragma unroll
  for (int j = 0; j < FN; ++j) {
    const float4 cs = *reinterpret_cast<const float4*>(s_cs + c0 + j * 16 + lq * 4);
    const float4 bs = *reinterpret_cast<const float4*>(s_cs + BN + c0 + j * 16 + lq * 4);
#pragma unroll
    for (int i = 0; i < FM; ++i) {
      const float2 st = s_ln[r0 + i * 16 + lr];
      const float mean = st.x, rstd = st.y;
      f32x4& a = acc[i][j];
      a[0] = __builtin_fmaf(rstd, a[0] - mean * cs.x, bs.x); a[1] = __builtin_fmaf(rstd, a[1] - mean * cs.y, bs.y);
      a[2] = __builtin_fmaf(rstd, a[2] - mean * cs.z, bs.z); a[3] = __builtin_fmaf(rstd, a[3] - mean * cs.w, bs.w);
    }
  }
}

template <int BM, int BN, int WM, int WN, int EM, bool LNF = false>
__global__ __launch_bounds__(WM* WN * 64) void gemm_kernel(const GemmDesc p) {
  constexpr int NT = WM * WN * 64;
  constexpr int TM = BM / WM, TN = BN / WN;
  constexpr int FM = TM / 16, FN = TN / 16;
  constexpr int A_PER = BM * 8 / NT, B_PER = BN * 8 / NT;
  constexpr int ROWS_PER_PASS = NT / 8;
  constexpr int A_BYTES = BM * 128, B_BYTES = BN * 128, STAGE = A_BYTES + B_BYTES;
  static_assert(A_PER >= 1 && B_PER >= 1, "tile too small for the thread count");

  extern __shared__ __attribute__((aligned(16))) char smem[];
  short2* s_taps = reinterpret_cast<short2*>(smem + 2 * STAGE);

  const int tid = threadIdx.x;
  const int tiles_n = (p.N + BN - 1) / BN;
  const int tn = blockIdx.x % tiles_n, tm = blockIdx.x / tiles_n;
  const int z = blockIdx.y;
  const int zo = z / p.Zi, zi = z - zo * p.Zi;
  const act_t* __restrict__ Ab = p.A + zo * p.sAo + zi * p.sAi;
  const act_t* __restrict__ Wb = p.W + zo * p.sWo + zi * p.sWi;
  const long long coff = zo * p.sCo + zi * p.sCi;

  if (tid < DMX_MAX_TAPS) s_taps[tid] = make_short2(p.tdy[tid], p.tdx[tid]);
  float2* s_ln = reinterpret_cast<float2*>(smem + 2 * STAGE + DMX_MAX_TAPS * 4);
  float* s_cs = reinterpret_cast<float*>(smem + 2 * STAGE + DMX_MAX_TAPS * 4 + BM * 8);
  int m0t = tm * BM, mlim = p.M;
  if constexpr (EM == 5 || EM == 6) {
    const int P = p.Hq * p.Wq;
    if (P % TM != 0) {
      const int tpi = (P + BM - 1) / BM, b = tm / tpi;
      m0t = b * P + (tm - b * tpi) * BM;
      mlim = (b + 1) * P;
    }
  }
  if constexpr (LNF) ln_prologue<BM, BN, NT>(p, m0t, tn * BN, s_ln, s_cs);

  const int cc = tid & 7, r0 = tid >> 3;
  const int cpt = p.Ci >> 3;
  const int HqWq = p.Hq * p.Wq;
  const act_t* a_base[A_PER];
  int a_iy[A_PER], a_ix[A_PER];
#pragma unroll
  for (int i = 0; i < A_PER; ++i) {
    const int m = m0t + r0 + i * ROWS_PER_PASS;
    if (m < mlim) {
      const int b = m / HqWq, rem = m - b * HqWq;
      const int qy = rem / p.Wq, qx = rem - qy * p.Wq;
      a_base[i] = Ab + (long long)b * p.Hi * p.Wi * p.lda;
      a_iy[i] = qy * p.sy;
      a_ix[i] = qx * p.sx;
    } else {
      a_base[i] = Ab;
      a_iy[i] = -(1 << 20);
      a_ix[i] = 0;
    }
  }
  const act_t* w_base[B_PER];
  bool w_ok[B_PER];
#pragma unroll
  for (int i = 0; i < B_PER; ++i) {
    const int n = tn * BN + r0 + i * ROWS_PER_PASS;
    w_ok[i] = n < p.N;
    w_base[i] = Wb + (long long)(w_ok[i] ? n : 0) * p.ldw;
  }
  __syncthreads();

  uint4 ra[A_PER], rb[B_PER];
  const int kchunks = p.K >> 3;
  auto load_tile = [&](int ks) {
    const int kc = ks * 8 + cc;
    const int tap = kc / cpt;
    const int cin = (kc - tap * cpt) << 3;
    const bool kval = kc < kchunks;
    const short2 t = s_taps[tap & (DMX_MAX_TAPS - 1)];
#pragma unroll
    for (int i = 0; i < A_PER; ++i) {
      const int iy = a_iy[i] + t.x, ix = a_ix[i] + t.y;
      const bool ok = kval && (unsigned)iy < (unsigned)p.Hi && (unsigned)ix < (unsigned)p.Wi;
      ra[i] = make_uint4(0, 0, 0, 0);
      if (ok) ra[i] = *reinterpret_cast<const uint4*>(a_base[i] + (long long)(iy * p.Wi + ix) * p.lda + cin);
    }
#pragma unroll
    for (int i = 0; i < B_PER; ++i) {
      rb[i] = make_uint4(0, 0, 0, 0);
      if (kval && w_ok[i]) rb[i] = *reinterpret_cast<const uint4*>(w_base[i] + (kc << 3));
    }
  };
  auto store_tile = [&](int buf) {
    char* sa = smem + buf * STAGE;
    char* sb = sa + A_BYTES;
#pragma unroll
    for (int i = 0; i < A_PER; ++i) {
      const int r = r0 + i * ROWS_PER_PASS;
      *reinterpret_cast<uint4*>(sa + r * 128 + ((cc ^ (r & 7)) << 4)) = ra[i];
    }
#pragma unroll
    for (int i = 0; i < B_PER; ++i) {
      const int r = r0 + i * ROWS_PER_PASS;
      *reinterpret_cast<uint4*>(sb + r * 128 + ((cc ^ (r & 7)) << 4)) = rb[i];
    }
  };

  const int wave = tid >> 6, lane = tid & 63;
  const int wm = wave / WN, wn = wave - wm * WN;
  const int lr = lane & 15, lq = lane >> 4;

  f32x4 acc[FM][FN];
  if (p.flags & EPI_BIASINIT) {
#pragma unroll
    for (int j = 0; j < FN; ++j) {
      const int n = tn * BN + wn * TN + j * 16 + lq * 4;
      float bb[4];
#pragma unroll
      for (int e = 0; e < 4; ++e) bb[e] = n + e < p.N ? p.bias[n + e] : 0.f;
#pragma unroll
      for (int i = 0; i < FM; ++i) acc[i][j] = f32x4{bb[0], bb[1], bb[2], bb[3]};
    }
  } else {
#pragma unroll
    for (int i = 0; i < FM; ++i)
#pragma unroll
      for (int j = 0; j < FN; ++j) acc[i][j] = f32x4{0.f, 0.f, 0.f, 0.f};
  }

  const int nk = (p.K + BK - 1) / BK;
  load_tile(0);
  store_tile(0);
  __syncthreads();

  for (int ks = 0; ks < nk; ++ks) {
    const int cur = ks & 1;
    if (ks + 1 < nk) load_tile(ks + 1);
    const char* sa = smem + cur * STAGE + (wm * TM + lr) * 128;
    const char* sb = smem + cur * STAGE + A_BYTES + (wn * TN + lr) * 128;
#pragma unroll
    for (int kk = 0; kk < 2; ++kk) {
      const int sw = ((kk * 4 + lq) ^ (lr & 7)) << 4;
      frag8_t af[FM], wf[FN];
#pragma unroll
      for (int i = 0; i < FM; ++i) af[i] = *reinterpret_cast<const frag8_t*>(sa + i * 16 * 128 + sw);
#pragma unroll
      for (int j = 0; j < FN; ++j) wf[j] = *reinterpret_cast<const frag8_t*>(sb + j * 16 * 128 + sw);
#pragma unroll
      for (int i = 0; i < FM; ++i)
#pragma unroll
        for (int j = 0; j < FN; ++j)
          acc[i][j] = DMX_MFMA16(wf[j], af[i], acc[i][j]);
    }
    if (ks + 1 < nk) store_tile(cur ^ 1);
    __syncthreads();
  }
  if constexpr (LNF) ln_apply<FM, FN, BN>(acc, s_ln, s_cs, wm * TM, wn * TN, lr, lq);

  if ((p.flags & EPI_F32OUT) || ((p.N | p.ldc | p.ldr | p.ldx | p.ldc2) & 7)) {
    gemm_epilogue<FM, FN>(p, acc, m0t + wm * TM, tn * BN + wn * TN, lr, lq, coff, HqWq);
  } else {
    constexpr int EPI_CH = EpiChunk<FM>::CH;
    constexpr int EPI_WAVE_BYTES = EPI_CH * (FN * 32 + 16) + EPI_CH * 12;
    static_assert(EPI_WAVE_BYTES * WM * WN <= 2 * (BM + BN) * 128, "epilogue staging does not fit the stage buffers");
    gemm_epilogue_lds<FM, FN, EM>(p, acc, m0t + wm * TM, tn * BN + wn * TN, lane, coff, HqWq, smem + wave * EPI_WAVE_BYTES, mlim);
  }
}

constexpr unsigned OOB = 0x80000000u;

#ifdef DMX_GEMM_STAMPS
__device__ unsigned long long g_gemm_stamps[8192 * 6];
#define DMX_GSTAMP(i) do { gstamp_v[i] = wall_clock64(); } while (0)
#else
#define DMX_GSTAMP(i) do { } while (0)
#endif

constexpr int SLAB_HALO = 64;

template <int BM, int BN, int WM, int WN, int NSTAGE, int EM, bool LNF = false, int SLAB = 0>
__device__ __forceinline__ void glds_tile(const GemmDesc& p, char* smem, const int m0, const int tn, const int mlim) {
  constexpr int NW = WM * WN;
  constexpr int TM = BM / WM, TN = BN / WN;
  constexpr int FM = TM / 16, FN = TN / 16;
  constexpr int A_ISS = BM / 8 / NW, B_ISS = BN / 8 / NW;
  constexpr int A_BYTES = BM * 128, B_BYTES = BN * 128, STAGE = A_BYTES + B_BYTES;
  static_assert(A_ISS >= 1 && B_ISS >= 1, "tile too small");
  constexpr int SLAB_BYTES = (BM + SLAB_HALO) * 128, SLAB_ISS = (BM + SLAB_HALO) / 8 / NW;
  constexpr int W_OFF = SLAB > 0 ? 2 * SLAB_BYTES : A_BYTES, W_STAGE = SLAB > 0 ? B_BYTES : STAGE;
  static_assert(SLAB == 0 || (NSTAGE == 2 && !LNF && (BM + SLAB_HALO) % (8 * NW) == 0 && TM % 8 == 0), "slab loop: two stages, whole pieces per wave");

  constexpr int PER = SLAB > 0 ? B_ISS + SLAB : A_ISS + B_ISS;
  constexpr int KEEP = (NSTAGE - 2) * PER;

  const int tid = threadIdx.x;
  const int wave = __builtin_amdgcn_readfirstlane(tid >> 6), lane = tid & 63;
#ifdef DMX_GEMM_STAMPS
  unsigned long long gstamp_v[5] = {0, 0, 0, 0, 0};
#endif
  DMX_GSTAMP(0);
  const int z = blockIdx.y;
  const int zo = z / p.Zi, zi = z - zo * p.Zi;
  const act_t* Ab = p.A + zo * p.sAo + zi * p.sAi;
  const act_t* Wb = p.W + zo * p.sWo + zi * p.sWi;
  const int nsplit = p.ksplit > 1 ? p.ksplit : 1, sp = blockIdx.z;
  const long long coff = zo * p.sCo + zi * p.sCi + (nsplit > 1 ? (long long)sp * p.M * p.N : 0ll);
  const __amdgpu_buffer_rsrc_t rsA = __builtin_amdgcn_make_buffer_rsrc(const_cast<act_t*>(Ab), 0, OOB, 0x00020000);
  const __amdgpu_buffer_rsrc_t rsW = __builtin_amdgcn_make_buffer_rsrc(const_cast<act_t*>(Wb), 0, (unsigned)p.N * (unsigned)p.ldw * 2u, 0x00020000);

  int tapreg = 0;
#pragma unroll
  for (int j = 0; j < DMX_MAX_TAPS; ++j)
    if (lane == j) tapreg = (int)(unsigned char)p.tdy[j] | ((int)(unsigned char)p.tdx[j] << 8);

  const int lrow = lane >> 3, cc = (lane & 7) ^ lrow;
  const int cpt = p.Ci >> 3;
  const int HqWq = p.Hq * p.Wq;
  const unsigned lda2 = (unsigned)p.lda * 2u;
  unsigned a_lin[A_ISS], a_mask2[(A_ISS + 1) / 2];
  int s_ix0 = 0, s_lo = 0;
  unsigned s_lin0 = 0u;
  if constexpr (SLAB > 0) {
    s_lo = 127;
    for (int t = 0; t < p.ntaps; ++t) {
      const int dx = (int)(signed char)((__builtin_amdgcn_readlane(tapreg, t) >> 8) & 0xff);
      s_lo = dx < s_lo ? dx : s_lo;
    }
    const int b = m0 / HqWq;
    s_ix0 = m0 - b * HqWq + s_lo + wave * 8 + lrow;
    s_lin0 = ((unsigned)b * (unsigned)p.Wi + (unsigned)s_ix0) * lda2 + ((unsigned)cc << 4);
  } else {
    int r_iy[A_ISS], r_ix[A_ISS];
    unsigned r_mask[A_ISS];
#pragma unroll
    for (int i = 0; i < A_ISS; ++i) {
      const int m = m0 + (i * NW + wave) * 8 + lrow;
      r_mask[i] = 0u; a_lin[i] = 0u;
      r_iy[i] = -(1 << 20); r_ix[i] = 0;
      if (m < mlim) {
        int b = 0, qy = 0, qx = m;
        if (!(p.Hq == 1 && p.Wq >= p.M)) {
          b = m / HqWq; const int rem = m - b * HqWq;
          qy = rem / p.Wq; qx = rem - qy * p.Wq;
        }
        r_iy[i] = qy * p.sy; r_ix[i] = qx * p.sx;
        a_lin[i] = (unsigned)b * (unsigned)(p.Hi * p.Wi) * lda2 + (unsigned)(r_iy[i] * p.Wi + r_ix[i]) * lda2 + ((unsigned)cc << 4);
      }
    }
    for (int t = 0; t < p.ntaps; ++t) {
      const int tv = __builtin_amdgcn_readlane(tapreg, t);
      const int dy = (int)(signed char)(tv & 0xff), dx = (int)(signed char)((tv >> 8) & 0xff);
#pragma unroll
      for (int i = 0; i < A_ISS; ++i)
        if ((unsigned)(r_iy[i] + dy) < (unsigned)p.Hi && (unsigned)(r_ix[i] + dx) < (unsigned)p.Wi) r_mask[i] |= 1u << t;
    }
#pragma unroll
    for (int i = 0; i < (A_ISS + 1) / 2; ++i) a_mask2[i] = 0u;
#pragma unroll
    for (int i = 0; i < A_ISS; ++i) a_mask2[i >> 1] |= r_mask[i] << ((i & 1) * 16);
  }
  const unsigned ldw2 = (unsigned)p.ldw * 2u;
  const unsigned w_row = (unsigned)(tn * BN + wave * 8 + lrow) * ldw2;
  const unsigned w_step = (unsigned)(NW * 8) * ldw2;

  const int kchunks = p.K >> 3;
  const bool tap_inner = (p.Ci & 63) == 0 || p.ntaps == 1;
  const int cgroups = (p.Ci + 63) >> 6;
  const int nk_all = (p.K + BK - 1) / BK;
  const int ks_per = (nk_all + nsplit - 1) / nsplit;
  const int ks0 = sp * ks_per, ks1 = ks0 + ks_per < nk_all ? ks0 + ks_per : nk_all;
  int i_cg = ks0 / p.ntaps, i_tp = ks0 - i_cg * p.ntaps;
  bool q_kval = false;
  int q_tp = 0;
  unsigned q_adel = 0, q_wdel = 0;
  char* q_base = nullptr;
  int c_tp = 0, c_cg = 0;
  int q_pi0 = 0;
  bool q_sval = false;
  unsigned q_sdel = 0;
  char* q_sbase = nullptr;
  auto slab_piece = [&](int pi, char* base, unsigned del) {
    const int ix = s_ix0 + pi * (NW * 8);
    const unsigned voff = (unsigned)ix < (unsigned)p.Wi ? s_lin0 + (unsigned)(pi * (NW * 8)) * lda2 + del : OOB;
    __builtin_amdgcn_raw_ptr_buffer_load_lds(rsA, (__attribute__((address_space(3))) void*)(base + (pi * NW + wave) * 1024), 16, voff, 0, 0, 0);
  };
  auto issue_begin = [&](int ksl, int stage) {
    if constexpr (SLAB > 0) {
      const int tp = __builtin_amdgcn_readfirstlane(i_tp), cgi = __builtin_amdgcn_readfirstlane(i_cg);
      q_base = smem + W_OFF + stage * W_STAGE;
      q_kval = cgi < cgroups;
      q_wdel = (unsigned)(tp * cpt + cgi * 8 + cc) << 4;
      if (++i_tp == p.ntaps) { i_tp = 0; ++i_cg; }
      const int ctp = __builtin_amdgcn_readfirstlane(c_tp), ccg = __builtin_amdgcn_readfirstlane(c_cg);
      q_pi0 = ctp * SLAB;
      q_sval = ccg + 1 < cgroups;
      q_sdel = (unsigned)(ccg + 1) << 7;
      q_sbase = smem + ((ccg + 1) & 1) * SLAB_BYTES;
      return;
    }
    q_base = smem + stage * STAGE;
    if (tap_inner) {
      const int tp = __builtin_amdgcn_readfirstlane(i_tp), cgi = __builtin_amdgcn_readfirstlane(i_cg);
      q_kval = cgi < cgroups && ksl + ks0 < ks1 && cgi * 8 + cc < cpt;
      const int tv = __builtin_amdgcn_readlane(tapreg, tp);
      const int dy = (int)(signed char)(tv & 0xff), dx = (int)(signed char)((tv >> 8) & 0xff);
      q_tp = tp;
      q_adel = (unsigned)((dy * p.Wi + dx) * (int)lda2) + ((unsigned)cgi << 7);
      q_wdel = (unsigned)(tp * cpt + cgi * 8 + cc) << 4;
      if (++i_tp == p.ntaps) { i_tp = 0; ++i_cg; }
    } else {
      const int ks = ksl + ks0;
      const int kc = ks * 8 + cc;
      const int tap = kc / cpt;
      q_kval = kc < kchunks && ks < ks1;
      const int tv = __builtin_amdgcn_ds_bpermute((tap & (DMX_MAX_TAPS - 1)) << 2, tapreg);
      const int dy = (int)(signed char)(tv & 0xff), dx = (int)(signed char)((tv >> 8) & 0xff);
      q_tp = tap & (DMX_MAX_TAPS - 1);
      q_adel = (unsigned)((dy * p.Wi + dx) * (int)lda2) + ((unsigned)(kc - tap * cpt) << 4) - ((unsigned)cc << 4);
      q_wdel = (unsigned)kc << 4;
    }
  };
  auto issue_one = [&](auto I) {
    constexpr int i = decltype(I)::value;
    if constexpr (SLAB > 0 && i >= B_ISS) {
      const int pi = q_pi0 + (i - B_ISS);
      if (pi < SLAB_ISS && q_sval) slab_piece(pi, q_sbase, q_sdel);
    } else if constexpr (SLAB > 0) {
      const unsigned voff = q_kval ? w_row + (unsigned)i * w_step + q_wdel : OOB;
      __builtin_amdgcn_raw_ptr_buffer_load_lds(rsW, (__attribute__((address_space(3))) void*)(q_base + (i * NW + wave) * 1024), 16, voff, 0, 0, 0);
    } else if constexpr (i < A_ISS) {
      const bool ok = q_kval && ((a_mask2[i >> 1] >> ((i & 1) * 16 + q_tp)) & 1u);
      const unsigned voff = ok ? a_lin[i] + q_adel : OOB;
      __builtin_amdgcn_raw_ptr_buffer_load_lds(rsA, (__attribute__((address_space(3))) void*)(q_base + (i * NW + wave) * 1024), 16, voff, 0, 0, 0);
    } else {
      constexpr int j = i - A_ISS;
      const unsigned voff = q_kval ? w_row + (unsigned)j * w_step + q_wdel : OOB;
      __builtin_amdgcn_raw_ptr_buffer_load_lds(rsW, (__attribute__((address_space(3))) void*)(q_base + A_BYTES + (j * NW + wave) * 1024), 16, voff, 0, 0, 0);
    }
  };
  auto issue = [&](int ksl, int stage) {
    issue_begin(ksl, stage);
    static_for<0, PER>(issue_one);
  };

  const int wm = wave / WN, wn = wave - wm * WN;
  const int lr = lane & 15, lq = lane >> 4;
  f32x4 acc[FM][FN];
  if (p.flags & EPI_BIASINIT) {
#pragma unroll
    for (int j = 0; j < FN; ++j) {
      const int n = tn * BN + wn * TN + j * 16 + lq * 4;
      const float4 bb = n < p.N ? *reinterpret_cast<const float4*>(p.bias + n) : make_float4(0.f, 0.f, 0.f, 0.f);
#pragma unroll
      for (int i = 0; i < FM; ++i) acc[i][j] = f32x4{bb.x, bb.y, bb.z, bb.w};
    }
  } else {
#pragma unroll
    for (int i = 0; i < FM; ++i)
#pragma unroll
      for (int j = 0; j < FN; ++j) acc[i][j] = f32x4{0.f, 0.f, 0.f, 0.f};
  }

  const int nk = ks1 > ks0 ? ks1 - ks0 : 0;
  if constexpr (SLAB > 0) {
    static_for<0, SLAB_ISS>([&](auto PI) { slab_piece(decltype(PI)::value, smem, 0u); });
    issue_begin(0, 0);
    static_for<0, B_ISS>(issue_one);
  } else {
#pragma unroll
    for (int s = 0; s < NSTAGE - 1; ++s) issue(s, s);
  }
  float2* s_ln = reinterpret_cast<float2*>(smem + NSTAGE * STAGE);
  float* s_cs = reinterpret_cast<float*>(smem + NSTAGE * STAGE + BM * 8);
  if constexpr (LNF) ln_prologue<BM, BN, NW * 64>(p, m0, tn * BN, s_ln, s_cs);
  asm volatile("s_waitcnt vmcnt(%0)" ::"n"(KEEP) : "memory");
  __builtin_amdgcn_s_barrier();
  DMX_GSTAMP(1);

  constexpr int NS = 2 * FM;
  constexpr int P0 = FN + 2;
  constexpr bool ROOMY = FM * FN * 4 + 4 * FM + 8 * FN + 64 <= 256;
  constexpr bool STAGGER = NW == 8 && FM >= 2 && (ROOMY || DMX_DEF_BIG > 0);
  constexpr int DEF = ROOMY ? FM : (DMX_DEF_BIG > 0 ? (DMX_DEF_BIG < FM ? DMX_DEF_BIG : FM) : 1);
  constexpr int LOWN = NS - DEF;
  static_assert(DEF <= FM && DEF >= 1, "carried steps must all be kk = 1 steps");
  static_assert(SLAB == 0 || !STAGGER, "the slab loop exists for the unstaggered 320-row tile");
  frag8_t wf0[FN], wf1[FN], af[NS];
#define DMX_DSR(dst, addr, off) asm volatile("ds_read_b128 %0, %1 offset:%2" : "=v"(dst) : "v"(addr), "n"(off))
  auto kloop = [&](auto LAGT) {
    constexpr bool LAG = decltype(LAGT)::value;
    int cur = 0, nxt = NSTAGE - 1;
    auto mfma_step = [&wf0, &wf1, &af, &acc](auto ST) {
      constexpr int st = decltype(ST)::value;
      constexpr int kk = st / FM, i = st - kk * FM;
#pragma unroll
      for (int j = 0; j < FN; ++j) acc[i][j] = DMX_MFMA16(kk ? wf1[j] : wf0[j], af[st], acc[i][j]);
      __builtin_amdgcn_sched_barrier(0);
    };
    for (int ks = 0; ks < nk; ++ks) {
      unsigned aA0, aA1, aB0, aB1;
      if constexpr (SLAB > 0) {
        const int tp = __builtin_amdgcn_readfirstlane(c_tp), cg = __builtin_amdgcn_readfirstlane(c_cg);
        const int dx = (int)(signed char)((__builtin_amdgcn_readlane(tapreg, tp) >> 8) & 0xff);
        const int row = wm * TM + lr + (dx - s_lo);
        const char* sa = smem + (cg & 1) * SLAB_BYTES + row * 128;
        const char* sb = smem + W_OFF + cur * W_STAGE + (wn * TN + lr) * 128;
        const unsigned a0 = (unsigned)(size_t)(__attribute__((address_space(3))) const char*)(sa);
        const unsigned b0 = (unsigned)(size_t)(__attribute__((address_space(3))) const char*)(sb);
        aA0 = a0 + (((0 * 4 + lq) ^ (row & 7)) << 4); aA1 = a0 + (((1 * 4 + lq) ^ (row & 7)) << 4);
        aB0 = b0 + (((0 * 4 + lq) ^ (lr & 7)) << 4); aB1 = b0 + (((1 * 4 + lq) ^ (lr & 7)) << 4);
      } else {
        const char* sa = smem + cur * STAGE + (wm * TM + lr) * 128;
        const char* sb = smem + cur * STAGE + A_BYTES + (wn * TN + lr) * 128;
        const unsigned a0 = (unsigned)(size_t)(__attribute__((address_space(3))) const char*)(sa);
        const unsigned b0 = (unsigned)(size_t)(__attribute__((address_space(3))) const char*)(sb);
        const unsigned sw0 = ((0 * 4 + lq) ^ (lr & 7)) << 4, sw1 = ((1 * 4 + lq) ^ (lr & 7)) << 4;
        aA0 = a0 + sw0; aA1 = a0 + sw1; aB0 = b0 + sw0; aB1 = b0 + sw1;
      }
      __builtin_amdgcn_sched_barrier(0);
      constexpr bool P0_LATE = LAG && DEF < FM;
      auto prologue_reads = [&wf0, &af, aA0, aA1, aB0]() {
        static_for<0, FN>([&wf0, aB0](auto J) { constexpr int j = decltype(J)::value; DMX_DSR(wf0[j], aB0, j * 2048); });
        DMX_DSR(af[0], aA0, 0);
        if constexpr (FM > 1) { DMX_DSR(af[1], aA0, 2048); } else { DMX_DSR(af[1], aA1, 0); }
      };
      if constexpr (!P0_LATE) prologue_reads();
      auto read_step = [&wf1, &af, aA0, aA1, aB1](auto ST) {
        constexpr int st = decltype(ST)::value;
        if constexpr (st + 2 < NS) {
          constexpr int s2 = st + 2, k2 = s2 / FM, i2 = s2 - k2 * FM;
          if constexpr (k2 == 0) { DMX_DSR(af[s2], aA0, i2 * 2048); } else { DMX_DSR(af[s2], aA1, i2 * 2048); }
        }
        if constexpr (LAG && st >= LOWN - (DEF - 2) && st < LOWN) {
          constexpr int s3 = st + DEF, i3 = s3 - FM;
          DMX_DSR(af[s3], aA1, i3 * 2048);
        }
        constexpr int w_lo = st < FM ? st * FN / FM : 0, w_hi = st < FM ? (st + 1) * FN / FM : 0;
        static_for<w_lo, w_hi>([&wf1, aB1](auto J) { constexpr int j = decltype(J)::value; DMX_DSR(wf1[j], aB1, j * 2048); });
      };
      auto wait_step = [](auto ST) {
        constexpr int st = decltype(ST)::value;
        constexpr auto r = [](int t) {
          const int trickle = t < FM ? (t + 1) * FN / FM - t * FN / FM : 0;
          return (t + 2 < NS ? 1 : 0) + (LAG && t >= LOWN - (DEF - 2) && t < LOWN ? 1 : 0) + trickle;
        };
        constexpr auto issued_through = [r](int t) { int n = P0; for (int q = 0; q <= t; ++q) n += r(q); return n; };
        constexpr int total = issued_through(st);
        constexpr int pos_af = st == 0 ? FN + 1 : (st == 1 ? FN + 2 : issued_through(st - 3 < 0 ? -1 : st - 3) + 1);
        constexpr int pos_w = st < FM ? FN : issued_through(FM - 1);
        constexpr int need = pos_af > pos_w ? pos_af : pos_w;
        asm volatile("s_waitcnt lgkmcnt(%0)" ::"n"(total - need) : "memory");
        __builtin_amdgcn_sched_barrier(0);
      };
      __builtin_amdgcn_sched_barrier(0);
      issue_begin(ks + NSTAGE - 1, nxt);
      __builtin_amdgcn_sched_barrier(0);
      constexpr int SPREAD = NS / 2 > 0 ? NS / 2 : 1;
      if constexpr (LAG) {
        if (ks > 0) {
          static_for<LOWN, NS>([&](auto ST) {
            constexpr int st = decltype(ST)::value;
            mfma_step(ST);
            static_for<(st - LOWN) * PER / DEF, (st - LOWN + 1) * PER / DEF>(issue_one);
            __builtin_amdgcn_sched_barrier(0);
          });
        } else {
          static_for<0, PER>(issue_one);
          __builtin_amdgcn_sched_barrier(0);
        }
        if constexpr (P0_LATE) { prologue_reads(); __builtin_amdgcn_sched_barrier(0); }
        static_for<0, LOWN>([&](auto ST) {
          read_step(ST);
          wait_step(ST);
          mfma_step(ST);
        });
      } else {
        static_for<0, NS>([&](auto ST) {
          constexpr int st = decltype(ST)::value;
          read_step(ST);
          wait_step(ST);
          mfma_step(ST);
          if constexpr (st < SPREAD) {
            static_for<st * PER / SPREAD, (st + 1) * PER / SPREAD>(issue_one);
            __builtin_amdgcn_sched_barrier(0);
          }
        });
      }
      asm volatile("s_waitcnt vmcnt(%0)\n\ts_waitcnt lgkmcnt(0)" ::"n"(KEEP) : "memory");
      __builtin_amdgcn_s_barrier();
      cur = cur + 1 == NSTAGE ? 0 : cur + 1;
      nxt = nxt + 1 == NSTAGE ? 0 : nxt + 1;
      if constexpr (SLAB > 0) { if (++c_tp == p.ntaps) { c_tp = 0; ++c_cg; } }
    }
    if constexpr (LAG) {
      __builtin_amdgcn_sched_barrier(0);
      if (nk > 0) static_for<LOWN, NS>(mfma_step);
    }
  };
  if constexpr (STAGGER) {
    if (wave >= NW / 2) kloop(std::true_type{}); else kloop(std::false_type{});
  } else {
    kloop(std::false_type{});
  }
#undef DMX_DSR
  asm volatile("s_waitcnt vmcnt(0)" ::: "memory");
  __builtin_amdgcn_s_barrier();
  DMX_GSTAMP(2);
  if constexpr (LNF) ln_apply<FM, FN, BN>(acc, s_ln, s_cs, wm * TM, wn * TN, lr, lq);
  if ((p.flags & EPI_F32OUT) || ((p.N | p.ldc | p.ldr | p.ldx | p.ldc2) & 7)) {
    gemm_epilogue<FM, FN>(p, acc, m0 + wm * TM, tn * BN + wn * TN, lr, lq, coff, HqWq);
  } else {
    constexpr int EPI_CH = EpiChunk<FM>::CH;
    constexpr int EPI_WAVE_BYTES = EPI_CH * (FN * 32 + 16) + EPI_CH * 12;
    static_assert(EPI_WAVE_BYTES * WM * WN <= 2 * (BM + BN) * 128, "epilogue staging does not fit the stage buffers");
    gemm_epilogue_lds<FM, FN, EM>(p, acc, m0 + wm * TM, tn * BN + wn * TN, lane, coff, HqWq, smem + wave * EPI_WAVE_BYTES, mlim);
  }
#ifdef DMX_GEMM_STAMPS
  DMX_GSTAMP(3);
  asm volatile("s_waitcnt vmcnt(0)" ::: "memory");
  DMX_GSTAMP(4);
  {
    const int wg = blockIdx.x + gridDim.x * (blockIdx.y + gridDim.y * blockIdx.z);
    if (tid == NW * 64 - 64 && wg < 8192) {
      unsigned hw, xcc;
      asm volatile("s_getreg_b32 %0, hwreg(HW_REG_HW_ID)" : "=s"(hw));
      asm volatile("s_getreg_b32 %0, hwreg(HW_REG_XCC_ID)" : "=s"(xcc));
#pragma unroll
      for (int i = 0; i < 5; ++i) g_gemm_stamps[wg * 6 + i] = gstamp_v[i];
      g_gemm_stamps[wg * 6 + 5] = ((unsigned long long)(xcc & 0xf) << 32) | hw;
    }
  }
#endif
}

__device__ __forceinline__ int xcd_remap(int bid) {
  const int nwg = gridDim.x, q = nwg >> 3, r = nwg & 7, xcd = bid & 7, loc = bid >> 3;
  return (xcd < r ? xcd * (q + 1) : r * (q + 1) + (xcd - r) * q) + loc;
}

template <int BM, int BN, int WM, int WN, int NSTAGE, int EM, bool LNF = false, int SLAB = 0>
__global__ __launch_bounds__(WM* WN * 64) void gemm_glds_kernel(const GemmDesc p) {
  extern __shared__ __attribute__((aligned(16))) char smem[];
  const int tiles_n = (p.N + BN - 1) / BN;
  const int bid = xcd_remap(blockIdx.x);
  int m0 = (bid / tiles_n) * BM, mlim = p.M;
  if constexpr (EM == 5 || EM == 6) {
    const int P = p.Hq * p.Wq;
    if (P % (BM / WM) != 0) {
      const int tpi = (P + BM - 1) / BM, tm = bid / tiles_n, b = tm / tpi;
      m0 = b * P + (tm - b * tpi) * BM;
      mlim = (b + 1) * P;
    }
  }
  if constexpr (SLAB > 0) {
    const int P = p.Wq, tpi = (P + BM - 1) / BM, tm = bid / tiles_n, b = tm / tpi;
    m0 = b * P + (tm - b * tpi) * BM;
    mlim = (b + 1) * P;
  }
  glds_tile<BM, BN, WM, WN, NSTAGE, EM, LNF, SLAB>(p, smem, m0, bid % tiles_n, mlim);
}

template <int BM, int BN, int WM, int WN, int NSTAGE, int EM, bool LNF = false, int SLAB = 0>
int launch_glds_t(const GemmDesc& d, hipStream_t stream) {
  constexpr int NT = WM * WN * 64;
  constexpr int SMEM = SLAB > 0 ? 2 * (BM + SLAB_HALO + BN) * 128 : NSTAGE * (BM + BN) * 128 + (LNF ? BM * 8 + BN * 8 : 0);
  static_assert(SMEM <= 160 * 1024, "tile ring exceeds the 160 KiB of LDS");
  static bool attr_set = false;
  if (!attr_set) {
    hipFuncSetAttribute(reinterpret_cast<const void*>(&gemm_glds_kernel<BM, BN, WM, WN, NSTAGE, EM, LNF, SLAB>),
                        hipFuncAttributeMaxDynamicSharedMemorySize, SMEM);
    attr_set = true;
  }
  long long tiles = (long long)cdiv(d.M, BM) * cdiv(d.N, BN);
  if constexpr (EM == 5 || EM == 6) {
    const int P = d.Hq * d.Wq;
    if (P % (BM / WM) != 0) tiles = (long long)(d.M / P) * cdiv(P, BM) * cdiv(d.N, BN);
  }
  if constexpr (SLAB > 0) tiles = (long long)(d.M / d.Wq) * cdiv(d.Wq, BM) * cdiv(d.N, BN);
  dim3 grid((unsigned)tiles, (unsigned)d.Z, (unsigned)(d.ksplit > 1 ? d.ksplit : 1));
  static const bool bias_init = getenv("DMX_NO_BIAS_INIT") == nullptr;
  if (bias_init && (d.flags & EPI_BIAS) && d.bias && !(d.flags & (EPI_MASK | EPI_MASKBITS | EPI_SOFTBWD | EPI_LNFOLD))) {
    GemmDesc q = d;
    q.flags = (q.flags & ~EPI_BIAS) | EPI_BIASINIT;
    hipLaunchKernelGGL((gemm_glds_kernel<BM, BN, WM, WN, NSTAGE, EM, LNF, SLAB>), grid, dim3(NT), SMEM, stream, q);
    return hipGetLastError() == hipSuccess ? DMX_OK : DMX_ERR_LAUNCH;
  }
  hipLaunchKernelGGL((gemm_glds_kernel<BM, BN, WM, WN, NSTAGE, EM, LNF, SLAB>), grid, dim3(NT), SMEM, stream, d);
  return hipGetLastError() == hipSuccess ? DMX_OK : DMX_ERR_LAUNCH;
}
template <int BM, int BN, int WM, int WN, int EM, bool LNF = false>
int launch_cfg_t(const GemmDesc& d, hipStream_t stream) {
  constexpr int NT = WM * WN * 64;
  constexpr int SMEM = 2 * (BM + BN) * 128 + DMX_MAX_TAPS * 4 + (LNF ? BM * 8 + BN * 8 : 0);
  static bool attr_set = false;
  if (!attr_set) {
    hipFuncSetAttribute(reinterpret_cast<const void*>(&gemm_kernel<BM, BN, WM, WN, EM, LNF>),
                        hipFuncAttributeMaxDynamicSharedMemorySize, SMEM);
    attr_set = true;
  }
  long long tiles = (long long)cdiv(d.M, BM) * cdiv(d.N, BN);
  if constexpr (EM == 5 || EM == 6) {
    const int P = d.Hq * d.Wq;
    if (P % (BM / WM) != 0) tiles = (long long)(d.M / P) * cdiv(P, BM) * cdiv(d.N, BN);
  }
  dim3 grid((unsigned)tiles, (unsigned)d.Z, 1);
  static const bool bias_init = getenv("DMX_NO_BIAS_INIT") == nullptr;
  if (bias_init && (d.flags & EPI_BIAS) && d.bias && !(d.flags & (EPI_MASK | EPI_MASKBITS | EPI_SOFTBWD | EPI_LNFOLD))) {
    GemmDesc q = d;
    q.flags = (q.flags & ~EPI_BIAS) | EPI_BIASINIT;
    hipLaunchKernelGGL((gemm_kernel<BM, BN, WM, WN, EM, LNF>), grid, dim3(NT), SMEM, stream, q);
    return hipGetLastError() == hipSuccess ? DMX_OK : DMX_ERR_LAUNCH;
  }
  hipLaunchKernelGGL((gemm_kernel<BM, BN, WM, WN, EM, LNF>), grid, dim3(NT), SMEM, stream, d);
  return hipGetLastError() == hipSuccess ? DMX_OK : DMX_ERR_LAUNCH;
}
}
```

Baseline: 26.97 steps/s (weak scaling: one step advances a batch of 8 clips on one GPU; value = K / wall x 1 GPU(s)).

## Read K-major GEMM operands via LDS transpose loads instead of explicit transposes

Adds K-major operand modes to the async-LDS GEMM tile. The kernel stages K-major rows into LDS and reads MFMA fragments with ds_read_b64_tr_b16 transposing loads. Attention forward (P·V) and the VAE attention backward GEMMs now pass V, dO, K, Q, P and dS directly instead of first running separate transpose kernels into scratch buffers, which removes several full-tensor transpose round trips and their memory. In exchange these GEMMs are pinned to the 256x256 tile with no split-K, each fragment read needs twice as many LDS instructions, and some shapes fall back or are rejected.

```diff
diff --git a/diffmusic_amd/_lib.py b/diffmusic_amd/_lib.py
--- a/diffmusic_amd/_lib.py
+++ b/diffmusic_amd/_lib.py
@@ -58,6 +58,7 @@
 EPI_BIAS, EPI_ROWBIAS, EPI_RESID, EPI_ACCUM, EPI_MASK, EPI_LRELU2, EPI_TANH, EPI_F32OUT, EPI_NO_C, EPI_RESID_INV, EPI_MASKBITS, EPI_BITS2, EPI_SOFTBWD = \
     1, 2, 4, 8, 16, 32, 64, 128, 256, 512, 1024, 2048, 4096
 EPI_GEGLU, EPI_LNFOLD, EPI_ROWSTATS, EPI_GNSTATS, EPI_GNBWD = 8192, 16384, 32768, 65536, 131072
+GEMM_A_KMAJOR, GEMM_B_KMAJOR = 1 << 19, 1 << 20
 
 _SIGS = {
     "dmx_abi_version": (C.c_int, []),
diff --git a/diffmusic_amd/csrc/blocks.h b/diffmusic_amd/csrc/blocks.h
--- a/diffmusic_amd/csrc/blocks.h
+++ b/diffmusic_amd/csrc/blocks.h
@@ -205,6 +205,8 @@
   }
 };
 
+inline bool attn_kmajor() { return getenv("DMX_NO_KMAJOR") == nullptr; }
+
 inline int attention_core(Ctx& cx, const act_t* q, const act_t* k, const act_t* v, act_t* o, int B, int Nq, int Nk, int C,
                           int heads, act_t* P_keep, const float* colbias, int ldq = 0, int ldk = 0, int ldv = 0) {
   if (ldq <= 0) ldq = C;
@@ -225,7 +227,8 @@
     return DMX_OK;
   }
   act_t* Pm = P_keep ? P_keep : A.bf((size_t)Z * Nq * Nkp);
-  act_t* vT = A.bf((size_t)Z * dh * Nkp);
+  const bool v_kmajor = attn_kmajor() && Nkp == Nk;
+  act_t* vT = v_kmajor ? nullptr : A.bf((size_t)Z * dh * Nkp);
   GemmBatch gb;
   gb.Z = Z; gb.Zi = heads;
   gb.sAo = (long long)Nq * ldq; gb.sAi = dh;
@@ -234,15 +237,21 @@
   Epi e; e.alpha = scale;
   CRUN(gemm_nt(q, ldq, k, ldk, Pm, Nkp, Nq, Nk, dh, e, gb, cx.st));
   CRUN(dmx_softmax_act(Pm, Pm, colbias, (long long)Z * Nq, Nk, Nkp, heads * Nq, cx.st));
-  if (Nkp != Nk && !cx.dry) (void)hipMemsetAsync(vT, 0, (size_t)Z * dh * Nkp * sizeof(act_t), cx.st);
-  CRUN(dmx_transpose(v, vT, Nk, dh, ldv, Nkp, Z, heads, (long long)Nk * ldv, dh, (long long)heads * dh * Nkp, (long long)dh * Nkp, cx.st));
   GemmBatch g2;
   g2.Z = Z; g2.Zi = heads;
   g2.sAo = (long long)heads * Nq * Nkp; g2.sAi = (long long)Nq * Nkp;
-  g2.sBo = (long long)heads * dh * Nkp; g2.sBi = (long long)dh * Nkp;
   g2.sCo = (long long)Nq * C; g2.sCi = dh;
   Epi e2;
-  CRUN(gemm_nt(Pm, Nkp, vT, Nkp, o, C, Nq, dh, Nkp, e2, g2, cx.st));
+  if (v_kmajor) {
+    g2.sBo = (long long)Nk * ldv; g2.sBi = dh;
+    e2.flags = GEMM_B_KMAJOR;
+    CRUN(gemm_nt(Pm, Nkp, v, ldv, o, C, Nq, dh, Nk, e2, g2, cx.st));
+  } else {
+    if (Nkp != Nk && !cx.dry) (void)hipMemsetAsync(vT, 0, (size_t)Z * dh * Nkp * sizeof(act_t), cx.st);
+    CRUN(dmx_transpose(v, vT, Nk, dh, ldv, Nkp, Z, heads, (long long)Nk * ldv, dh, (long long)heads * dh * Nkp, (long long)dh * Nkp, cx.st));
+    g2.sBo = (long long)heads * dh * Nkp; g2.sBi = (long long)dh * Nkp;
+    CRUN(gemm_nt(Pm, Nkp, vT, Nkp, o, C, Nq, dh, Nkp, e2, g2, cx.st));
+  }
   A.release(mk);
   return DMX_OK;
 }
@@ -308,12 +317,13 @@
     if ((long long)B * N * C >= (1ll << 29)) { dmx_set_error("vae attention backward: B*h*w*C >= 2^29 elements unsupported"); return DMX_ERR_SHAPE; }
     const float scale = 1.0f / sqrtf((float)C);
     const size_t mk = A.mark();
+    const bool km = attn_kmajor();
     act_t* go = A.bf((size_t)B * N * C);
-    act_t* goT = A.bf((size_t)B * N * C);
-    act_t* PT = A.bf((size_t)B * N * N);
+    act_t* goT = km ? nullptr : A.bf((size_t)B * N * C);
+    act_t* PT = km ? nullptr : A.bf((size_t)B * N * N);
     float* delta = A.f32((size_t)B * N);
     act_t* dS = A.bf((size_t)B * N * N);
-    act_t* T1 = A.bf((size_t)B * N * C);
+    act_t* T1 = km ? nullptr : A.bf((size_t)B * N * C);
     act_t* gq = A.bf((size_t)B * N * C);
     act_t* gk = A.bf((size_t)B * N * C);
     act_t* gv = A.bf((size_t)B * N * C);
@@ -327,15 +337,23 @@
       Epi es; es.flags = EPI_SOFTBWD; es.X = Pm; es.rowbias = delta; es.alpha = scale;
       CRUN(gemm_nt(go, C, v, C, dS, N, N, N, C, es, gb, st));
     }
-    CRUN(dmx_transpose(Pm, PT, N, N, N, N, B, 1, (long long)N * N, 0, (long long)N * N, 0, st));
-    CRUN(dmx_transpose(go, goT, N, C, C, N, B, 1, (long long)N * C, 0, (long long)N * C, 0, st));
     gb.sAo = (long long)N * N; gb.sBo = (long long)N * C; gb.sCo = (long long)N * C;
-    CRUN(gemm_nt(PT, N, goT, N, gv, C, N, C, N, e, gb, st));
-    CRUN(dmx_transpose(k, T1, N, C, C, N, B, 1, (long long)N * C, 0, (long long)N * C, 0, st));
-    CRUN(gemm_nt(dS, N, T1, N, gq, C, N, C, N, e, gb, st));
-    CRUN(dmx_transpose(dS, PT, N, N, N, N, B, 1, (long long)N * N, 0, (long long)N * N, 0, st));
-    CRUN(dmx_transpose(q, T1, N, C, C, N, B, 1, (long long)N * C, 0, (long long)N * C, 0, st));
-    CRUN(gemm_nt(PT, N, T1, N, gk, C, N, C, N, e, gb, st));
+    if (km) {
+      Epi eab; eab.flags = GEMM_A_KMAJOR | GEMM_B_KMAJOR;
+      CRUN(gemm_nt(Pm, N, go, C, gv, C, N, C, N, eab, gb, st));
+      Epi eb; eb.flags = GEMM_B_KMAJOR;
+      CRUN(gemm_nt(dS, N, k, C, gq, C, N, C, N, eb, gb, st));
+      CRUN(gemm_nt(dS, N, q, C, gk, C, N, C, N, eab, gb, st));
+    } else {
+      CRUN(dmx_transpose(Pm, PT, N, N, N, N, B, 1, (long long)N * N, 0, (long long)N * N, 0, st));
+      CRUN(dmx_transpose(go, goT, N, C, C, N, B, 1, (long long)N * C, 0, (long long)N * C, 0, st));
+      CRUN(gemm_nt(PT, N, goT, N, gv, C, N, C, N, e, gb, st));
+      CRUN(dmx_transpose(k, T1, N, C, C, N, B, 1, (long long)N * C, 0, (long long)N * C, 0, st));
+      CRUN(gemm_nt(dS, N, T1, N, gq, C, N, C, N, e, gb, st));
+      CRUN(dmx_transpose(dS, PT, N, N, N, N, B, 1, (long long)N * N, 0, (long long)N * N, 0, st));
+      CRUN(dmx_transpose(q, T1, N, C, C, N, B, 1, (long long)N * C, 0, (long long)N * C, 0, st));
+      CRUN(gemm_nt(PT, N, T1, N, gk, C, N, C, N, e, gb, st));
+    }
     Epi ea; ea.flags = EPI_ACCUM;
     CRUN(linear_bwd(to_q, gq, C, gxn, C, (long long)B * N, e, st));
     CRUN(linear_bwd(to_k, gk, C, gxn, C, (long long)B * N, ea, st));
diff --git a/diffmusic_amd/csrc/dmx_common.h b/diffmusic_amd/csrc/dmx_common.h
--- a/diffmusic_amd/csrc/dmx_common.h
+++ b/diffmusic_amd/csrc/dmx_common.h
@@ -94,7 +94,9 @@
   EPI_GNSTATS = 65536,
   EPI_GNBWD = 131072,
   EPI_BIASINIT = 262144,
-  EPI_SOFTBWD = 4096
+  EPI_SOFTBWD = 4096,
+  GEMM_A_KMAJOR = 524288,
+  GEMM_B_KMAJOR = 1048576
 };
 
 struct GemmDesc {
@@ -145,6 +147,7 @@
 int dmx_gemm_launch_ln(int cfg, const GemmDesc& d, hipStream_t stream);
 int dmx_gemm_launch_rowstats(int cfg, const GemmDesc& d, hipStream_t stream);
 int dmx_gemm_launch_gnstats(int cfg, const GemmDesc& d, hipStream_t stream, int* gn_rows);
+int dmx_gemm_launch_kmajor(const GemmDesc& d, hipStream_t stream);
 bool dmx_prof_is_active();
 bool dmx_gemm_slab_ok(const GemmDesc& d);
 int dmx_gemm_last_cfg();
diff --git a/diffmusic_amd/csrc/gemm_conv.hip b/diffmusic_amd/csrc/gemm_conv.hip
--- a/diffmusic_amd/csrc/gemm_conv.hip
+++ b/diffmusic_amd/csrc/gemm_conv.hip
@@ -1,4 +1,6 @@
 #include "gemm_tile.h"
+
+void dmx_set_error(const char* fmt, ...);
 
 namespace {
 template <int BM, int BN, int WM, int WN, int NSTAGE>
@@ -111,6 +113,7 @@
   }
 }
 int launch_dispatch(const GemmDesc& d, hipStream_t stream, int* gn_rows) {
+  if (d.flags & (GEMM_A_KMAJOR | GEMM_B_KMAJOR)) { g_last_cfg = 1; return dmx_gemm_launch_kmajor(d, stream); }
   const bool gl = glds_ok(d);
   if (d.flags & EPI_SOFTBWD) return gl ? launch_by_cfg(1, d, stream, gn_rows) : DMX_ERR_SHAPE;
   if (d.tile_cfg >= 1 && d.tile_cfg <= 22 && ((d.tile_cfg > 2 && d.tile_cfg < 7) || gl)) return launch_by_cfg(d.tile_cfg, d, stream, gn_rows);
@@ -264,7 +267,7 @@
 
 int splitk_plan(const GemmDesc& d, int* tile) {
   static const bool off = getenv("DMX_NO_SPLITK") != nullptr;
-  if (off || !g_splitk_ws || d.Z != 1 || !glds_ok(d)) return 1;
+  if (off || !g_splitk_ws || d.Z != 1 || !glds_ok(d) || (d.flags & (GEMM_A_KMAJOR | GEMM_B_KMAJOR))) return 1;
   if (d.flags & (EPI_ACCUM | EPI_F32OUT | EPI_TANH | EPI_MASKBITS | EPI_BITS2 | EPI_SOFTBWD | EPI_GEGLU | EPI_LNFOLD | EPI_ROWSTATS)) return 1;
   if (!(d.osy == 1 && d.osx == 1 && d.ooy == 0 && d.oox == 0 && d.Ho == d.Hq && d.Wo == d.Wq)) return 1;
   if ((d.N & 7) || (d.ldc & 3)) return 1;
@@ -332,6 +335,23 @@
   if ((d.Ci & 7) || (d.N & 3) || (d.K & 7) || (d.lda & 7) || (d.ldw & 7) || (d.ldc & 3)) return DMX_ERR_SHAPE;
   if (d.ntaps < 1 || d.ntaps > DMX_MAX_TAPS || d.K != d.ntaps * d.Ci) return DMX_ERR_SHAPE;
   if (d.Z < 1 || d.Zi < 1) return DMX_ERR_SHAPE;
+  if (d.flags & (GEMM_A_KMAJOR | GEMM_B_KMAJOR)) {
+    const bool ak = (d.flags & GEMM_A_KMAJOR) != 0, wk = (d.flags & GEMM_B_KMAJOR) != 0;
+    if (d.ntaps != 1 || d.Hi != 1 || d.Hq != 1 || d.Wq < d.M || d.sx != 1 || d.tdx[0] != 0 || d.tdy[0] != 0 ||
+        !(d.osy == 1 && d.osx == 1 && d.ooy == 0 && d.oox == 0 && d.Ho == d.Hq && d.Wo == d.Wq)) {
+      dmx_set_error("K-major GEMM operands: plain or batched GEMMs only (ntaps = %d, Hq = %d)", d.ntaps, d.Hq);
+      return DMX_ERR_SHAPE;
+    }
+    if (d.tile_cfg >= 100 || d.ksplit > 1) { dmx_set_error("K-major GEMM operands: no split-K (tile_cfg = %d)", d.tile_cfg); return DMX_ERR_SHAPE; }
+    if (d.tile_cfg != 0 && d.tile_cfg != 1) { dmx_set_error("K-major GEMM operands run on tile 1 (256 x 256), not tile %d", d.tile_cfg); return DMX_ERR_SHAPE; }
+    if (d.flags & (EPI_SOFTBWD | EPI_GEGLU | EPI_MASKBITS | EPI_BITS2 | EPI_LNFOLD | EPI_ROWSTATS | EPI_GNSTATS | EPI_GNBWD)) {
+      dmx_set_error("K-major GEMM operands: epilogue flags 0x%x have no K-major kernel", d.flags);
+      return DMX_ERR_SHAPE;
+    }
+    if ((ak && (d.M & 7)) || (wk && (d.N & 7))) { dmx_set_error("a K-major GEMM operand needs its contiguous extent %% 8 == 0 (M = %d, N = %d)", d.M, d.N); return DMX_ERR_SHAPE; }
+    const long long a_el = ak ? (long long)d.K * d.lda : (long long)d.M * d.lda, w_el = wk ? (long long)d.K * d.ldw : ((long long)d.N + 512) * d.ldw;
+    if (a_el >= (1ll << 29) || w_el >= (1ll << 29)) { dmx_set_error("K-major GEMM operands: an operand of 2^29 elements or more is unsupported"); return DMX_ERR_SHAPE; }
+  }
   if ((d.flags & EPI_LRELU2) && !(d.act_slope >= 0.f && d.act_slope <= 1.f)) return DMX_ERR_SHAPE;
   if ((d.flags & EPI_RESID_INV) && !(d.resid_inv_slope >= 1.f)) return DMX_ERR_SHAPE;
   if (d.flags & EPI_SOFTBWD) {
diff --git a/diffmusic_amd/csrc/gemm_kmajor.hip b/diffmusic_amd/csrc/gemm_kmajor.hip
--- /dev/null
+++ b/diffmusic_amd/csrc/gemm_kmajor.hip
@@ -0,0 +1,11 @@
+#include "gemm_tile.h"
+
+int dmx_gemm_launch_kmajor(const GemmDesc& d, hipStream_t stream) {
+  const bool ak = (d.flags & GEMM_A_KMAJOR) != 0, wk = (d.flags & GEMM_B_KMAJOR) != 0;
+  GemmDesc q = d;
+  q.flags &= ~(GEMM_A_KMAJOR | GEMM_B_KMAJOR);
+  if (ak && wk) return launch_glds_t<256, 256, 2, 4, 2, 0, false, 0, true, true>(q, stream);
+  if (ak) return launch_glds_t<256, 256, 2, 4, 2, 0, false, 0, true, false>(q, stream);
+  if (wk) return launch_glds_t<256, 256, 2, 4, 2, 0, false, 0, false, true>(q, stream);
+  return DMX_ERR_SHAPE;
+}
diff --git a/diffmusic_amd/csrc/gemm_tile.h b/diffmusic_amd/csrc/gemm_tile.h
--- a/diffmusic_amd/csrc/gemm_tile.h
+++ b/diffmusic_amd/csrc/gemm_tile.h
@@ -234,7 +234,7 @@
 
 constexpr int SLAB_HALO = 64;
 
-template <int BM, int BN, int WM, int WN, int NSTAGE, int EM, bool LNF = false, int SLAB = 0>
+template <int BM, int BN, int WM, int WN, int NSTAGE, int EM, bool LNF = false, int SLAB = 0, bool AK = false, bool WK = false>
 __device__ __forceinline__ void glds_tile(const GemmDesc& p, char* smem, const int m0, const int tn, const int mlim) {
   constexpr int NW = WM * WN;
   constexpr int TM = BM / WM, TN = BN / WN;
@@ -245,6 +245,9 @@
   constexpr int SLAB_BYTES = (BM + SLAB_HALO) * 128, SLAB_ISS = (BM + SLAB_HALO) / 8 / NW;
   constexpr int W_OFF = SLAB > 0 ? 2 * SLAB_BYTES : A_BYTES, W_STAGE = SLAB > 0 ? B_BYTES : STAGE;
   static_assert(SLAB == 0 || (NSTAGE == 2 && !LNF && (BM + SLAB_HALO) % (8 * NW) == 0 && TM % 8 == 0), "slab loop: two stages, whole pieces per wave");
+  static_assert(!(AK || WK) || (SLAB == 0 && !LNF && NW == 8 && EM == 0), "K-major operands: plain GEMMs on an 8-wave tile");
+  static_assert(!AK || (BM == 256 && FM <= 8), "a K-major A stage is 64 k-rows of 256 columns");
+  static_assert(!WK || (BN == 256 && FN <= 8), "a K-major W stage is 64 k-rows of 256 columns");
 
   constexpr int PER = SLAB > 0 ? B_ISS + SLAB : A_ISS + B_ISS;
   constexpr int KEEP = (NSTAGE - 2) * PER;
@@ -261,8 +264,10 @@
   const act_t* Wb = p.W + zo * p.sWo + zi * p.sWi;
   const int nsplit = p.ksplit > 1 ? p.ksplit : 1, sp = blockIdx.z;
   const long long coff = zo * p.sCo + zi * p.sCi + (nsplit > 1 ? (long long)sp * p.M * p.N : 0ll);
-  const __amdgpu_buffer_rsrc_t rsA = __builtin_amdgcn_make_buffer_rsrc(const_cast<act_t*>(Ab), 0, OOB, 0x00020000);
-  const __amdgpu_buffer_rsrc_t rsW = __builtin_amdgcn_make_buffer_rsrc(const_cast<act_t*>(Wb), 0, (unsigned)p.N * (unsigned)p.ldw * 2u, 0x00020000);
+  const __amdgpu_buffer_rsrc_t rsA = __builtin_amdgcn_make_buffer_rsrc(
+      const_cast<act_t*>(Ab), 0, AK ? ((unsigned)(p.K - 1) * (unsigned)p.lda + (unsigned)p.M) * 2u : OOB, 0x00020000);
+  const __amdgpu_buffer_rsrc_t rsW = __builtin_amdgcn_make_buffer_rsrc(
+      const_cast<act_t*>(Wb), 0, WK ? ((unsigned)(p.K - 1) * (unsigned)p.ldw + (unsigned)p.N) * 2u : (unsigned)p.N * (unsigned)p.ldw * 2u, 0x00020000);
 
   int tapreg = 0;
 #pragma unroll
@@ -276,7 +281,24 @@
   unsigned a_lin[A_ISS], a_mask2[(A_ISS + 1) / 2];
   int s_ix0 = 0, s_lo = 0;
   unsigned s_lin0 = 0u;
-  if constexpr (SLAB > 0) {
+  const int k_row0 = wave * 2 + (lane >> 5);
+  const int k_cc = (lane & 31) ^ ((((k_row0 & 3) | (((k_row0 >> 3) & 1) << 2))) << 1);
+  bool ak_ok = false, wk_ok = false;
+  unsigned ak_lin = 0u, wk_lin = 0u;
+  if constexpr (AK) {
+    ak_ok = m0 + k_cc * 8 < mlim;
+    ak_lin = (unsigned)k_row0 * lda2 + (unsigned)(m0 + k_cc * 8) * 2u;
+  }
+  if constexpr (WK) {
+    wk_ok = tn * BN + k_cc * 8 < p.N;
+    wk_lin = (unsigned)k_row0 * ((unsigned)p.ldw * 2u) + (unsigned)(tn * BN + k_cc * 8) * 2u;
+  }
+  if constexpr (AK) {
+#pragma unroll
+    for (int i = 0; i < A_ISS; ++i) a_lin[i] = 0u;
+#pragma unroll
+    for (int i = 0; i < (A_ISS + 1) / 2; ++i) a_mask2[i] = 0u;
+  } else if constexpr (SLAB > 0) {
     s_lo = 127;
     for (int t = 0; t < p.ntaps; ++t) {
       const int dx = (int)(signed char)((__builtin_amdgcn_readlane(tapreg, t) >> 8) & 0xff);
@@ -329,6 +351,7 @@
   bool q_kval = false;
   int q_tp = 0;
   unsigned q_adel = 0, q_wdel = 0;
+  int q_k0 = 0;
   char* q_base = nullptr;
   int c_tp = 0, c_cg = 0;
   int q_pi0 = 0;
@@ -363,6 +386,9 @@
       q_tp = tp;
       q_adel = (unsigned)((dy * p.Wi + dx) * (int)lda2) + ((unsigned)cgi << 7);
       q_wdel = (unsigned)(tp * cpt + cgi * 8 + cc) << 4;
+      if constexpr (AK || WK) q_k0 = (ksl + ks0 < ks1) ? cgi * 64 : p.K;
+      if constexpr (AK) q_adel = (unsigned)(cgi * 64) * lda2;
+      if constexpr (WK) q_wdel = (unsigned)(cgi * 64) * ldw2;
       if (++i_tp == p.ntaps) { i_tp = 0; ++i_cg; }
     } else {
       const int ks = ksl + ks0;
@@ -384,6 +410,15 @@
     } else if constexpr (SLAB > 0) {
       const unsigned voff = q_kval ? w_row + (unsigned)i * w_step + q_wdel : OOB;
       __builtin_amdgcn_raw_ptr_buffer_load_lds(rsW, (__attribute__((address_space(3))) void*)(q_base + (i * NW + wave) * 1024), 16, voff, 0, 0, 0);
+    } else if constexpr (AK && i < A_ISS) {
+      const bool ok = ak_ok && q_k0 + k_row0 + i * (2 * NW) < p.K;
+      const unsigned voff = ok ? ak_lin + q_adel + (unsigned)(i * 2 * NW) * lda2 : OOB;
+      __builtin_amdgcn_raw_ptr_buffer_load_lds(rsA, (__attribute__((address_space(3))) void*)(q_base + (i * NW + wave) * 1024), 16, voff, 0, 0, 0);
+    } else if constexpr (WK && i >= A_ISS) {
+      constexpr int j = i - A_ISS;
+      const bool ok = wk_ok && q_k0 + k_row0 + j * (2 * NW) < p.K;
+      const unsigned voff = ok ? wk_lin + q_wdel + (unsigned)(j * 2 * NW) * ldw2 : OOB;
+      __builtin_amdgcn_raw_ptr_buffer_load_lds(rsW, (__attribute__((address_space(3))) void*)(q_base + A_BYTES + (j * NW + wave) * 1024), 16, voff, 0, 0, 0);
     } else if constexpr (i < A_ISS) {
       const bool ok = q_kval && ((a_mask2[i >> 1] >> ((i & 1) * 16 + q_tp)) & 1u);
       const unsigned voff = ok ? a_lin[i] + q_adel : OOB;
@@ -443,6 +478,23 @@
   static_assert(SLAB == 0 || !STAGGER, "the slab loop exists for the unstaggered 320-row tile");
   frag8_t wf0[FN], wf1[FN], af[NS];
 #define DMX_DSR(dst, addr, off) asm volatile("ds_read_b128 %0, %1 offset:%2" : "=v"(dst) : "v"(addr), "n"(off))
+  typedef short dmx_s4 __attribute__((ext_vector_type(4)));
+#define DMX_DSRK(dst, addr, fi, kk)                                                                                                   \
+  do {                                                                                                                                \
+    dmx_s4 lo_, hi_;                                                                                                                  \
+    if constexpr ((fi) == 0) {                                                                                                        \
+      asm volatile("ds_read_b64_tr_b16 %0, %2 offset:%3\n\tds_read_b64_tr_b16 %1, %2 offset:%4"                                       \
+                   : "=&v"(lo_), "=&v"(hi_) : "v"(addr), "n"((kk) * 16384), "n"((kk) * 16384 + 2048));                                 \
+    } else {                                                                                                                          \
+      unsigned t_;                                                                                                                    \
+      asm volatile("v_xor_b32 %2, %4, %3\n\tds_read_b64_tr_b16 %0, %2 offset:%5\n\tds_read_b64_tr_b16 %1, %2 offset:%6"              \
+                   : "=&v"(lo_), "=&v"(hi_), "=&v"(t_) : "v"(addr), "n"((fi) << 5), "n"((kk) * 16384), "n"((kk) * 16384 + 2048));      \
+    }                                                                                                                                 \
+    dst = __builtin_bit_cast(frag8_t, __builtin_shufflevector(lo_, hi_, 0, 1, 2, 3, 4, 5, 6, 7));                                     \
+  } while (0)
+#define DMX_RD_A(dst, kk, i) do { if constexpr (AK) { DMX_DSRK(dst, aA0, i, kk); } else if constexpr ((kk) == 0) { DMX_DSR(dst, aA0, (i) * 2048); } else { DMX_DSR(dst, aA1, (i) * 2048); } } while (0)
+#define DMX_RD_W(dst, kk, j) do { if constexpr (WK) { DMX_DSRK(dst, aB0, j, kk); } else if constexpr ((kk) == 0) { DMX_DSR(dst, aB0, (j) * 2048); } else { DMX_DSR(dst, aB1, (j) * 2048); } } while (0)
+  constexpr int RA = AK ? 2 : 1, RW = WK ? 2 : 1;
   auto kloop = [&](auto LAGT) {
     constexpr bool LAG = decltype(LAGT)::value;
     int cur = 0, nxt = NSTAGE - 1;
@@ -472,39 +524,49 @@
         const unsigned b0 = (unsigned)(size_t)(__attribute__((address_space(3))) const char*)(sb);
         const unsigned sw0 = ((0 * 4 + lq) ^ (lr & 7)) << 4, sw1 = ((1 * 4 + lq) ^ (lr & 7)) << 4;
         aA0 = a0 + sw0; aA1 = a0 + sw1; aB0 = b0 + sw0; aB1 = b0 + sw1;
+        const unsigned kf5 = (unsigned)((lr >> 2) | ((lq & 1) << 2)) << 5, krow = (unsigned)(lq * 8 + (lr >> 2)) * 512u;
+        if constexpr (AK) {
+          const unsigned s0 = (unsigned)(size_t)(__attribute__((address_space(3))) const char*)(smem + cur * STAGE);
+          aA0 = s0 + krow + (((unsigned)(wm * TM * 2) | ((unsigned)(lr & 3) << 3)) ^ kf5); aA1 = aA0;
+        }
+        if constexpr (WK) {
+          const unsigned s0 = (unsigned)(size_t)(__attribute__((address_space(3))) const char*)(smem + cur * STAGE + A_BYTES);
+          aB0 = s0 + krow + (((unsigned)(wn * TN * 2) | ((unsigned)(lr & 3) << 3)) ^ kf5); aB1 = aB0;
+        }
       }
       __builtin_amdgcn_sched_barrier(0);
       constexpr bool P0_LATE = LAG && DEF < FM;
-      auto prologue_reads = [&wf0, &af, aA0, aA1, aB0]() {
-        static_for<0, FN>([&wf0, aB0](auto J) { constexpr int j = decltype(J)::value; DMX_DSR(wf0[j], aB0, j * 2048); });
-        DMX_DSR(af[0], aA0, 0);
-        if constexpr (FM > 1) { DMX_DSR(af[1], aA0, 2048); } else { DMX_DSR(af[1], aA1, 0); }
+      auto prologue_reads = [&wf0, &af, aA0, aA1, aB0, aB1]() {
+        static_for<0, FN>([&wf0, aB0, aB1](auto J) { constexpr int j = decltype(J)::value; DMX_RD_W(wf0[j], 0, j); });
+        DMX_RD_A(af[0], 0, 0);
+        if constexpr (FM > 1) { DMX_RD_A(af[1], 0, 1); } else { DMX_RD_A(af[1], 1, 0); }
       };
       if constexpr (!P0_LATE) prologue_reads();
-      auto read_step = [&wf1, &af, aA0, aA1, aB1](auto ST) {
+      auto read_step = [&wf1, &af, aA0, aA1, aB0, aB1](auto ST) {
         constexpr int st = decltype(ST)::value;
         if constexpr (st + 2 < NS) {
           constexpr int s2 = st + 2, k2 = s2 / FM, i2 = s2 - k2 * FM;
-          if constexpr (k2 == 0) { DMX_DSR(af[s2], aA0, i2 * 2048); } else { DMX_DSR(af[s2], aA1, i2 * 2048); }
+          DMX_RD_A(af[s2], k2, i2);
         }
         if constexpr (LAG && st >= LOWN - (DEF - 2) && st < LOWN) {
           constexpr int s3 = st + DEF, i3 = s3 - FM;
-          DMX_DSR(af[s3], aA1, i3 * 2048);
+          DMX_RD_A(af[s3], 1, i3);
         }
         constexpr int w_lo = st < FM ? st * FN / FM : 0, w_hi = st < FM ? (st + 1) * FN / FM : 0;
-        static_for<w_lo, w_hi>([&wf1, aB1](auto J) { constexpr int j = decltype(J)::value; DMX_DSR(wf1[j], aB1, j * 2048); });
+        static_for<w_lo, w_hi>([&wf1, aB0, aB1](auto J) { constexpr int j = decltype(J)::value; DMX_RD_W(wf1[j], 1, j); });
       };
       auto wait_step = [](auto ST) {
         constexpr int st = decltype(ST)::value;
         constexpr auto r = [](int t) {
           const int trickle = t < FM ? (t + 1) * FN / FM - t * FN / FM : 0;
-          return (t + 2 < NS ? 1 : 0) + (LAG && t >= LOWN - (DEF - 2) && t < LOWN ? 1 : 0) + trickle;
+          return RA * ((t + 2 < NS ? 1 : 0) + (LAG && t >= LOWN - (DEF - 2) && t < LOWN ? 1 : 0)) + RW * trickle;
         };
-        constexpr auto issued_through = [r](int t) { int n = P0; for (int q = 0; q <= t; ++q) n += r(q); return n; };
+        constexpr auto issued_through = [r](int t) { int n = RW * FN + RA * (P0 - FN); for (int q = 0; q <= t; ++q) n += r(q); return n; };
         constexpr int total = issued_through(st);
-        constexpr int pos_af = st == 0 ? FN + 1 : (st == 1 ? FN + 2 : issued_through(st - 3 < 0 ? -1 : st - 3) + 1);
-        constexpr int pos_w = st < FM ? FN : issued_through(FM - 1);
+        constexpr int pos_af = st == 0 ? RW * FN + RA : (st == 1 ? RW * FN + 2 * RA : issued_through(st - 3 < 0 ? -1 : st - 3) + RA);
+        constexpr int pos_w = st < FM ? RW * FN : issued_through(FM - 1);
         constexpr int need = pos_af > pos_w ? pos_af : pos_w;
+        static_assert(total - need <= 15, "lgkmcnt holds 4 bits");
         asm volatile("s_waitcnt lgkmcnt(%0)" ::"n"(total - need) : "memory");
         __builtin_amdgcn_sched_barrier(0);
       };
@@ -559,6 +621,9 @@
     kloop(std::false_type{});
   }
 #undef DMX_DSR
+#undef DMX_DSRK
+#undef DMX_RD_A
+#undef DMX_RD_W
   asm volatile("s_waitcnt vmcnt(0)" ::: "memory");
   __builtin_amdgcn_s_barrier();
   DMX_GSTAMP(2);
@@ -594,9 +659,9 @@
   return (xcd < r ? xcd * (q + 1) : r * (q + 1) + (xcd - r) * q) + loc;
 }
 
-template <int BM, int BN, int WM, int WN, int NSTAGE, int EM, bool LNF = false, int SLAB = 0>
+template <int BM, int BN, int WM, int WN, int NSTAGE, int EM, bool LNF = false, int SLAB = 0, bool AK = false, bool WK = false>
 __global__ __launch_bounds__(WM* WN * 64) void gemm_glds_kernel(const GemmDesc p) {
-  extern __shared__ __attribute__((aligned(16))) char smem[];
+  extern __shared__ __attribute__((aligned(1024))) char smem[];
   const int tiles_n = (p.N + BN - 1) / BN;
   const int bid = xcd_remap(blockIdx.x);
   int m0 = (bid / tiles_n) * BM, mlim = p.M;
@@ -613,17 +678,17 @@
     m0 = b * P + (tm - b * tpi) * BM;
     mlim = (b + 1) * P;
   }
-  glds_tile<BM, BN, WM, WN, NSTAGE, EM, LNF, SLAB>(p, smem, m0, bid % tiles_n, mlim);
-}
-
-template <int BM, int BN, int WM, int WN, int NSTAGE, int EM, bool LNF = false, int SLAB = 0>
+  glds_tile<BM, BN, WM, WN, NSTAGE, EM, LNF, SLAB, AK, WK>(p, smem, m0, bid % tiles_n, mlim);
+}
+
+template <int BM, int BN, int WM, int WN, int NSTAGE, int EM, bool LNF = false, int SLAB = 0, bool AK = false, bool WK = false>
 int launch_glds_t(const GemmDesc& d, hipStream_t stream) {
   constexpr int NT = WM * WN * 64;
   constexpr int SMEM = SLAB > 0 ? 2 * (BM + SLAB_HALO + BN) * 128 : NSTAGE * (BM + BN) * 128 + (LNF ? BM * 8 + BN * 8 : 0);
   static_assert(SMEM <= 160 * 1024, "tile ring exceeds the 160 KiB of LDS");
   static bool attr_set = false;
   if (!attr_set) {
-    hipFuncSetAttribute(reinterpret_cast<const void*>(&gemm_glds_kernel<BM, BN, WM, WN, NSTAGE, EM, LNF, SLAB>),
+    hipFuncSetAttribute(reinterpret_cast<const void*>(&gemm_glds_kernel<BM, BN, WM, WN, NSTAGE, EM, LNF, SLAB, AK, WK>),
                         hipFuncAttributeMaxDynamicSharedMemorySize, SMEM);
     attr_set = true;
   }
@@ -638,10 +703,10 @@
   if (bias_init && (d.flags & EPI_BIAS) && d.bias && !(d.flags & (EPI_MASK | EPI_MASKBITS | EPI_SOFTBWD | EPI_LNFOLD))) {
     GemmDesc q = d;
     q.flags = (q.flags & ~EPI_BIAS) | EPI_BIASINIT;
-    hipLaunchKernelGGL((gemm_glds_kernel<BM, BN, WM, WN, NSTAGE, EM, LNF, SLAB>), grid, dim3(NT), SMEM, stream, q);
+    hipLaunchKernelGGL((gemm_glds_kernel<BM, BN, WM, WN, NSTAGE, EM, LNF, SLAB, AK, WK>), grid, dim3(NT), SMEM, stream, q);
     return hipGetLastError() == hipSuccess ? DMX_OK : DMX_ERR_LAUNCH;
   }
-  hipLaunchKernelGGL((gemm_glds_kernel<BM, BN, WM, WN, NSTAGE, EM, LNF, SLAB>), grid, dim3(NT), SMEM, stream, d);
+  hipLaunchKernelGGL((gemm_glds_kernel<BM, BN, WM, WN, NSTAGE, EM, LNF, SLAB, AK, WK>), grid, dim3(NT), SMEM, stream, d);
   return hipGetLastError() == hipSuccess ? DMX_OK : DMX_ERR_LAUNCH;
 }
 template <int BM, int BN, int WM, int WN, int EM, bool LNF = false>
```

Measured after the change: 27.20 steps/s (weak scaling: one step advances a batch of 8 clips on one GPU; value = K / wall x 1 GPU(s)), median of 6. Within noise of the previous version (+0.9%).
